# kubeai-project/kubeai

Measured on AMD Instinct MI355X. Metric: output_tokens_per_s (k6 multi-turn chat), higher is better.
Workload: dtype fp8; 1 GPU; model=llama-3-8b, global_batch=40, seq_len=8192, parallelism=dp1, prefix_cache=True

## Files before the change

### kubeai_amd/csrc/attention_decode.hip

```cpp
#include <torch/extension.h>

#include <type_traits>

#include "attention_checks.h"
#include "attention_plan.h"
#include "common.h"
#include "dispatch.h"

namespace {

constexpr int kWaves = 2;
constexpr int kBlockThreads = kWaves * WAVE_SIZE;
constexpr int kBS = 16;
typedef __attribute__((ext_vector_type(2))) __bf16 bf16x2v;
constexpr int kPad = 8;

template <int G, typename CT = ushort, int HD = 128, bool CAP = false,
          bool RAW = false>
__launch_bounds__(kBlockThreads) __global__ void paged_decode_kernel(
    ushort* __restrict__ out,
    const ushort* __restrict__ q,
    std::conditional_t<RAW, CT*, const CT*> __restrict__ k_cache,
    std::conditional_t<RAW, CT*, const CT*> __restrict__ v_cache,
    const int32_t* __restrict__ block_tables,
    const int32_t* __restrict__ seq_lens,
    const float scale, const float softcap, const int window,
    const int n_kv, const int max_blocks,
    const int64_t q_stride, const int n_splits,
    float* __restrict__ part_o,
    float* __restrict__ part_ml,
    const ushort* __restrict__ k_new,
    const ushort* __restrict__ v_new,
    const int32_t* __restrict__ positions,
    const float* __restrict__ cos_sin,
    const int64_t* __restrict__ slot_mapping,
    const int64_t k_stride, const int64_t v_stride) {
  const int b = blockIdx.x / (n_kv * n_splits);
  const int rem = blockIdx.x % (n_kv * n_splits);
  const int kh = rem / n_splits;
  const int split = rem % n_splits;
  const int n_q = n_kv * G;
  const int wave = threadIdx.x / WAVE_SIZE;
  const int lane = threadIdx.x % WAVE_SIZE;
  const int L = seq_lens[b];
  int pos = 0;
  int64_t slot = -1;
  if constexpr (RAW) {
    pos = positions[b];
    slot = slot_mapping[b];
  }
  const int n_blocks = (L + kBS - 1) / kBS;
  const int w0 = (window > 0) ? max(0, L - window) : 0;
  const int blk_base = w0 / kBS;
  const int n_eff = n_blocks - blk_base;
  const int chunk = (n_eff + n_splits - 1) / n_splits;
  const int blk_lo = blk_base + split * chunk;
  const int blk_hi = min(n_blocks, blk_lo + chunk);

  constexpr int PARTS = HD / 32;
  constexpr int TOKP = 64 / PARTS;
  constexpr int EPL = HD / 64;
  __shared__ CT k_lds[kWaves][kBS][HD + kPad];
  __shared__ CT v_lds[kWaves][kBS][HD + kPad];
  __shared__ float merge_o[kWaves][G][HD];
  __shared__ float merge_ml[kWaves][G][2];

  const int tok_of = lane / PARTS;
  const int part = lane % PARTS;

  uint32_t q_pack[G][16];
  if constexpr (!RAW) {
#pragma unroll
    for (int g = 0; g < G; ++g) {
      const uint32_t* qp = reinterpret_cast<const uint32_t*>(
          q + (int64_t)b * q_stride + (int64_t)(kh * G + g) * HD + part * 32);
#pragma unroll
      for (int i = 0; i < 16; ++i) q_pack[g][i] = qp[i];
    }
  }

  const int32_t* bt = block_tables + (int64_t)b * max_blocks;
  const int first = blk_lo + wave;
  int64_t blk_first = 0;
  if constexpr (RAW) blk_first = bt[first < blk_hi ? first : 0];

  constexpr int HALF = HD / 2;
  constexpr int QV = G * HALF / 4;
  constexpr int QIT = (QV + WAVE_SIZE - 1) / WAVE_SIZE;
  ushort4_t q_lo[RAW ? QIT : 1], q_hi[RAW ? QIT : 1];
  float4_t q_c[RAW ? QIT : 1], q_s[RAW ? QIT : 1];
  constexpr int RV = HD / 8;
  ushort8 row_own, row_par;
  float4_t row_c[2], row_s[2];
  const bool row_hi = (lane % RV) >= RV / 2;
  if constexpr (RAW) {
    const float* cs = cos_sin + (int64_t)pos * HD;
#pragma unroll
    for (int it = 0; it < QIT; ++it) {
      const int idx = lane + it * WAVE_SIZE;
      if (QV % WAVE_SIZE == 0 || idx < QV) {
        const int g = idx / (HALF / 4);
        const int i = (idx % (HALF / 4)) * 4;
        const ushort* qh =
            q + (int64_t)b * q_stride + (int64_t)(kh * G + g) * HD + i;
        q_lo[it] = *reinterpret_cast<const ushort4_t*>(qh);
        q_hi[it] = *reinterpret_cast<const ushort4_t*>(qh + HALF);
        q_c[it] = *reinterpret_cast<const float4_t*>(cs + i);
        q_s[it] = *reinterpret_cast<const float4_t*>(cs + HALF + i);
      }
    }
    {
      const int e0 = (lane % RV) * 8;
      const ushort* row = ((lane / RV) % 2 == 0
                               ? k_new + (int64_t)b * k_stride
                               : v_new + (int64_t)b * v_stride) +
                          (int64_t)kh * HD;
      row_own = *reinterpret_cast<const ushort8*>(row + e0);
      row_par = *reinterpret_cast<const ushort8*>(
          row + (row_hi ? e0 - HALF : e0 + HALF));
      const int i = row_hi ? e0 - HALF : e0;
#pragma unroll
      for (int h = 0; h < 2; ++h) {
        row_c[h] = *reinterpret_cast<const float4_t*>(cs + i + 4 * h);
        row_s[h] = *reinterpret_cast<const float4_t*>(cs + HALF + i + 4 * h);
      }
    }
  }

  float m[G], l[G], o[G][EPL];
#pragma unroll
  for (int g = 0; g < G; ++g) {
    m[g] = -INFINITY;
    l[g] = 0.f;
#pragma unroll
    for (int e = 0; e < EPL; ++e) o[g][e] = 0.f;
  }

  using StageVec = std::conditional_t<sizeof(CT) == 2, ushort8, uint64_t>;
  constexpr int NS = (kBS * HD / 8) / WAVE_SIZE;
  StageVec stage_k[NS], stage_v[NS];
  typedef StageVec __attribute__((may_alias)) LdsVec;

  auto issue_tile = [&](const int64_t blk) {
    const CT* base_k = k_cache + ((blk * n_kv + kh) * kBS) * HD;
    const CT* base_v = v_cache + ((blk * n_kv + kh) * kBS) * HD;
    const StageVec* src_k = reinterpret_cast<const StageVec*>(base_k);
    const StageVec* src_v = reinterpret_cast<const StageVec*>(base_v);
#pragma unroll
    for (int i = 0; i < NS; ++i) {
      stage_k[i] = src_k[lane + i * WAVE_SIZE];
      stage_v[i] = src_v[lane + i * WAVE_SIZE];
    }
  };
  auto issue_loads = [&](int blk_i) { issue_tile(bt[blk_i]); };
  auto write_tile = [&]() {
#pragma unroll
    for (int i = 0; i < NS; ++i) {
      const int vec = lane + i * WAVE_SIZE;
      const int row = vec / (HD / 8);
      const int col = vec % (HD / 8);
      *reinterpret_cast<LdsVec*>(&k_lds[wave][row][col * 8]) = stage_k[i];
      *reinterpret_cast<LdsVec*>(&v_lds[wave][row][col * 8]) = stage_v[i];
    }
  };

  if (first < blk_hi) {
    if constexpr (RAW)
      issue_tile(blk_first);
    else
      issue_loads(first);
  }

  int row_blk = -1;
  StageVec row_vec{};
  if constexpr (RAW) {
    ushort* q_rot = reinterpret_cast<ushort*>(&merge_o[wave][0][0]);
#pragma unroll
    for (int it = 0; it < QIT; ++it) {
      const int idx = lane + it * WAVE_SIZE;
      if (QV % WAVE_SIZE == 0 || idx < QV) {
        const int g = idx / (HALF / 4);
        const int i = (idx % (HALF / 4)) * 4;
        ushort4_t r_lo, r_hi;
#pragma unroll
        for (int e = 0; e < 4; ++e) {
          ushort o1, o2;
          rope_rotate_pair(bf16_to_f32(q_lo[it][e]), bf16_to_f32(q_hi[it][e]),
                           q_c[it][e], q_s[it][e], o1, o2);
          r_lo[e] = o1;
          r_hi[e] = o2;
        }
        *reinterpret_cast<ushort4_t*>(q_rot + g * HD + i) = r_lo;
        *reinterpret_cast<ushort4_t*>(q_rot + g * HD + HALF + i) = r_hi;
      }
    }
#pragma unroll
    for (int g = 0; g < G; ++g) {
      const uint4* qp =
          reinterpret_cast<const uint4*>(q_rot + g * HD + part * 32);
#pragma unroll
      for (int i = 0; i < 4; ++i) {
        const uint4 t = qp[i];
        q_pack[g][4 * i] = t.x;
        q_pack[g][4 * i + 1] = t.y;
        q_pack[g][4 * i + 2] = t.z;
        q_pack[g][4 * i + 3] = t.w;
      }
    }

    const int new_blk = (L - 1) / kBS;
    const bool owner = slot >= 0 && L > 0 && new_blk >= blk_lo &&
                       new_blk < blk_hi && (new_blk - blk_lo) % kWaves == wave;
    if (owner) {
      row_blk = new_blk;
      if (lane < 2 * RV) {
        ushort8 row = row_own;
        if (lane < RV) {
#pragma unroll
          for (int e = 0; e < 8; ++e) {
            const float x_own = bf16_to_f32(row_own[e]);
            const float x_par = bf16_to_f32(row_par[e]);
            ushort o1, o2;
            rope_rotate_pair(row_hi ? x_par : x_own, row_hi ? x_own : x_par,
                             row_c[e / 4][e % 4], row_s[e / 4][e % 4], o1, o2);
            row[e] = row_hi ? o2 : o1;
          }
        }
        if constexpr (sizeof(CT) == 2) {
          row_vec = row;
        } else {
          row_vec = 0;
#pragma unroll
          for (int e = 0; e < 8; ++e)
            row_vec |= (uint64_t)f32_to_e5m2(bf16_to_f32((ushort)row[e]))
                       << (8 * e);
        }
        CT* dst = (lane < RV ? k_cache : v_cache) +
                  cache_row_offset(slot, kBS, n_kv, kh, HD) + (lane % RV) * 8;
        *reinterpret_cast<StageVec*>(dst) = row_vec;
      }
    }
  }
  if (first < blk_hi) write_tile();

  for (int blk_i = first; blk_i < blk_hi; blk_i += kWaves) {
    const int tile_start = blk_i * kBS;
    const int tile_len = min(kBS, L - tile_start);
    if (blk_i + kWaves < blk_hi) issue_loads(blk_i + kWaves);

    if constexpr (RAW) {
      if (blk_i == row_blk && lane < 2 * RV) {
        CT* dst = lane < RV ? &k_lds[wave][(L - 1) % kBS][lane * 8]
                            : &v_lds[wave][(L - 1) % kBS][(lane - RV) * 8];
        *reinterpret_cast<LdsVec*>(dst) = row_vec;
      }
    }

#pragma unroll
    for (int tp = 0; tp < kBS; tp += TOKP) {
      const int tok = tp + tok_of;
      float s[G];
#pragma unroll
      for (int g = 0; g < G; ++g) s[g] = 0.f;
      if constexpr (sizeof(CT) == 2) {
        const uint32_t* krow = reinterpret_cast<const uint32_t*>(
            &k_lds[wave][tok][part * 32]);
#pragma unroll
        for (int j = 0; j < 16; ++j) {
          const bf16x2v kk = __builtin_bit_cast(bf16x2v, krow[j]);
#pragma unroll
          for (int g = 0; g < G; ++g)
            s[g] = __builtin_amdgcn_fdot2_f32_bf16(
                kk, __builtin_bit_cast(bf16x2v, q_pack[g][j]), s[g], false);
        }
      } else {
        const uint32_t* krow = reinterpret_cast<const uint32_t*>(
            &k_lds[wave][tok][part * 32]);
#pragma unroll
        for (int j = 0; j < 8; ++j) {
          const uint32_t kk = krow[j];
          const floatx2 k01 = __builtin_amdgcn_cvt_pk_f32_bf8(kk, false);
          const floatx2 k23 = __builtin_amdgcn_cvt_pk_f32_bf8(kk, true);
#pragma unroll
          for (int g = 0; g < G; ++g) {
            const uint32_t qa = q_pack[g][2 * j];
            const uint32_t qb = q_pack[g][2 * j + 1];
            s[g] = fmaf(k01.x, bf16_to_f32((ushort)(qa & 0xffff)), s[g]);
            s[g] = fmaf(k01.y, bf16_to_f32((ushort)(qa >> 16)), s[g]);
            s[g] = fmaf(k23.x, bf16_to_f32((ushort)(qb & 0xffff)), s[g]);
            s[g] = fmaf(k23.y, bf16_to_f32((ushort)(qb >> 16)), s[g]);
          }
        }
      }
      float p[G];
      float rsum[G];
#pragma unroll
      for (int g = 0; g < G; ++g) {
#pragma unroll
        for (int off = 1; off < PARTS; off <<= 1)
          s[g] += __shfl_xor(s[g], off, 64);
        s[g] = (tok < tile_len && tile_start + tok >= w0) ? s[g] * scale
                                                          : -INFINITY;
        if constexpr (CAP) {
          if (s[g] != -INFINITY) s[g] = softcap * tanhf(s[g] / softcap);
        }
        float tmax = s[g];
#pragma unroll
        for (int off = PARTS; off < 64; off <<= 1)
          tmax = fmaxf(tmax, __shfl_xor(tmax, off, 64));
        const float m_new = fmaxf(m[g], tmax);
        if (m_new != m[g]) {
          const float corr = __expf(m[g] - m_new);
          l[g] *= corr;
#pragma unroll
          for (int e = 0; e < EPL; ++e) o[g][e] *= corr;
          m[g] = m_new;
        }
        p[g] = (s[g] == -INFINITY) ? 0.f : __expf(s[g] - m_new);
        rsum[g] = p[g];
#pragma unroll
        for (int off = 1; off < 64; off <<= 1)
          rsum[g] += __shfl_xor(rsum[g], off, 64);
        l[g] += rsum[g] * (1.0f / PARTS);
      }

#pragma unroll
      for (int t = tp; t < tp + TOKP; ++t) {
        if (t >= tile_len) break;
        float vv[EPL];
        if constexpr (sizeof(CT) == 2) {
#pragma unroll
          for (int e = 0; e < EPL; e += 2) {
            const uint32_t vr = *reinterpret_cast<const uint32_t*>(
                &v_lds[wave][t][EPL * lane + e]);
            vv[e] = bf16_to_f32((ushort)(vr & 0xffff));
            vv[e + 1] = bf16_to_f32((ushort)(vr >> 16));
          }
        } else {
#pragma unroll
          for (int e = 0; e < EPL; e += 2) {
            const uint32_t vr = *reinterpret_cast<const ushort*>(
                &v_lds[wave][t][EPL * lane + e]);
            const floatx2 vf = __builtin_amdgcn_cvt_pk_f32_bf8(vr, false);
            vv[e] = vf.x;
            vv[e + 1] = vf.y;
          }
        }
#pragma unroll
        for (int g = 0; g < G; ++g) {
          const float pt = __shfl(p[g], (t - tp) * PARTS, 64);
#pragma unroll
          for (int e = 0; e < EPL; ++e)
            o[g][e] = fmaf(pt, vv[e], o[g][e]);
        }
      }
    }

    if (blk_i + kWaves < blk_hi) write_tile();
  }

#pragma unroll
  for (int g = 0; g < G; ++g) {
#pragma unroll
    for (int e = 0; e < EPL; ++e) merge_o[wave][g][EPL * lane + e] = o[g][e];
    if (lane == 0) {
      merge_ml[wave][g][0] = m[g];
      merge_ml[wave][g][1] = l[g];
    }
  }
  __syncthreads();

  for (int g = wave; g < G; g += kWaves) {
    float m_star = -INFINITY;
#pragma unroll
    for (int w = 0; w < kWaves; ++w) m_star = fmaxf(m_star, merge_ml[w][g][0]);
    float l_star = 0.f, oo[EPL];
#pragma unroll
    for (int e = 0; e < EPL; ++e) oo[e] = 0.f;
    if (m_star != -INFINITY) {
#pragma unroll
      for (int w = 0; w < kWaves; ++w) {
        const float c = __expf(merge_ml[w][g][0] - m_star);
        l_star += merge_ml[w][g][1] * c;
#pragma unroll
        for (int e = 0; e < EPL; ++e)
          oo[e] += merge_o[w][g][EPL * lane + e] * c;
      }
    }
    const int head = kh * G + g;
    if (n_splits == 1) {
      const float inv_l = 1.0f / l_star;
      ushort* oh = out + ((int64_t)b * n_q + head) * HD;
#pragma unroll
      for (int e = 0; e < EPL; e += 2) {
        uint32_t packed =
            ((uint32_t)f32_to_bf16(oo[e + 1] * inv_l) << 16) |
            f32_to_bf16(oo[e] * inv_l);
        *reinterpret_cast<uint32_t*>(&oh[EPL * lane + e]) = packed;
      }
    } else {
      float* po = part_o + (((int64_t)b * n_q + head) * n_splits + split) * HD;
#pragma unroll
      for (int e = 0; e < EPL; ++e) po[EPL * lane + e] = oo[e];
      if (lane == 0) {
        float* pm = part_ml + (((int64_t)b * n_q + head) * n_splits + split) * 2;
        pm[0] = m_star;
        pm[1] = l_star;
      }
    }
  }
}

constexpr int kMergeSplitCapLo = 8;
constexpr int kMergeSplitCapHi = 16;

template <int N, int HD, int SCAP>
DEV_INLINE void merge_partials(const float* __restrict__ po,
                               const float* __restrict__ pml,
                               const int n_splits, uint32_t (&packed)[N / 2]) {
  typedef float __attribute__((ext_vector_type(N))) vecN;
  floatx2 ml[SCAP];
  vecN pv[SCAP];
#pragma unroll
  for (int s = 0; s < SCAP; ++s) {
    const int sc = min(s, n_splits - 1);
    ml[s] = *reinterpret_cast<const floatx2*>(pml + 2 * sc);
    pv[s] = *reinterpret_cast<const vecN*>(po + sc * HD);
  }
  __builtin_amdgcn_sched_barrier(0);
  float m_star = -INFINITY;
#pragma unroll
  for (int s = 0; s < SCAP; ++s)
    if (s < n_splits) m_star = fmaxf(m_star, ml[s].x);
  float l_star = 0.f, oo[N];
#pragma unroll
  for (int e = 0; e < N; ++e) oo[e] = 0.f;
#pragma unroll
  for (int s = 0; s < SCAP; ++s) {
    const bool use = s < n_splits && ml[s].x != -INFINITY;
    const float c = __expf(ml[s].x - m_star);
    l_star = use ? l_star + ml[s].y * c : l_star;
#pragma unroll
    for (int e = 0; e < N; ++e) oo[e] = use ? oo[e] + pv[s][e] * c : oo[e];
  }
  const float inv_l = 1.0f / l_star;
#pragma unroll
  for (int e = 0; e < N; e += 2)
    packed[e / 2] = ((uint32_t)f32_to_bf16(oo[e + 1] * inv_l) << 16) |
                    f32_to_bf16(oo[e] * inv_l);
}

template <int HD, int SCAP>
__global__ void decode_merge_kernel(
    ushort* __restrict__ out,
    const float* __restrict__ part_o,
    const float* __restrict__ part_ml,
    const int n_q, const int n_splits, const int64_t n_bh) {
  constexpr int EPL = HD / 64;
  const int64_t bh = (int64_t)blockIdx.x * (blockDim.x / WAVE_SIZE) +
                     threadIdx.x / WAVE_SIZE;
  if (bh >= n_bh) return;
  const int lane = threadIdx.x % WAVE_SIZE;
  uint32_t packed[EPL / 2];
  merge_partials<EPL, HD, SCAP>(part_o + bh * n_splits * HD + EPL * lane,
                                part_ml + bh * n_splits * 2, n_splits, packed);
  ushort* oh = out + bh * HD;
#pragma unroll
  for (int e = 0; e < EPL; e += 2)
    *reinterpret_cast<uint32_t*>(&oh[EPL * lane + e]) = packed[e / 2];
}

constexpr int kMergeVec = 4;
constexpr int kMergeMaxThreads = 1024;
constexpr int kMergeMaxPasses = 2;
constexpr int kMergeRowMax = kMergeMaxThreads * kMergeVec * kMergeMaxPasses;

template <int HD, int kPasses, int SCAP>
__launch_bounds__(kMergeMaxThreads) __global__ void decode_merge_fp8_kernel(
    ushort* __restrict__ out,
    unsigned char* __restrict__ out_fp8,
    float* __restrict__ out_scale,
    const float* __restrict__ part_o,
    const float* __restrict__ part_ml,
    const int n_q, const int n_splits) {
  __shared__ float red[16];
  const int b = blockIdx.x;
  const int row_len = n_q * HD;
  const int nvec = row_len / kMergeVec;
  ushort* orow = out + (int64_t)b * row_len;

  uint32_t packed[kPasses][kMergeVec / 2];
  float amax = 0.f;
#pragma unroll
  for (int it = 0; it < kPasses; ++it) {
    const int i = threadIdx.x + it * blockDim.x;
    if (i < nvec) {
      const int h = (i * kMergeVec) / HD;
      const int col = (i * kMergeVec) % HD;
      const int64_t bh = (int64_t)b * n_q + h;
      merge_partials<kMergeVec, HD, SCAP>(part_o + bh * n_splits * HD + col,
                                          part_ml + bh * n_splits * 2,
                                          n_splits, packed[it]);
      *reinterpret_cast<uint2*>(orow + i * kMergeVec) =
          make_uint2(packed[it][0], packed[it][1]);
#pragma unroll
      for (int e = 0; e < kMergeVec / 2; ++e) {
        const uint32_t pk = packed[it][e];
        amax = fmaxf(amax, fabsf(bf16_to_f32((ushort)(pk & 0xffff))));
        amax = fmaxf(amax, fabsf(bf16_to_f32((ushort)(pk >> 16))));
      }
    }
  }
  const float inv_scale = row_scale_fp8(amax, red, out_scale + b);
  unsigned char* frow = out_fp8 + (int64_t)b * row_len;
#pragma unroll
  for (int it = 0; it < kPasses; ++it) {
    const int i = threadIdx.x + it * blockDim.x;
    if (i < nvec) {
      uchar4 q4;
      const uint32_t p0 = packed[it][0], p1 = packed[it][1];
      q4.x = f32_to_fp8(bf16_to_f32((ushort)(p0 & 0xffff)) * inv_scale);
      q4.y = f32_to_fp8(bf16_to_f32((ushort)(p0 >> 16)) * inv_scale);
      q4.z = f32_to_fp8(bf16_to_f32((ushort)(p1 & 0xffff)) * inv_scale);
      q4.w = f32_to_fp8(bf16_to_f32((ushort)(p1 >> 16)) * inv_scale);
      *reinterpret_cast<uchar4*>(frow + i * kMergeVec) = q4;
    }
  }
}

}

void quant_fp8(torch::Tensor out, torch::Tensor out_scale, torch::Tensor x);

namespace {

struct RawQKV {
  torch::Tensor k, v, positions, cos_sin, slot_mapping;
};

void decode_impl(torch::Tensor out, const c10::optional<torch::Tensor>& out_fp8,
                 const c10::optional<torch::Tensor>& out_scale, torch::Tensor q,
                 torch::Tensor k_cache, torch::Tensor v_cache,
                 torch::Tensor block_tables, torch::Tensor seq_lens,
                 double scale, int64_t window, double softcap,
                 const RawQKV* raw = nullptr) {
  const AttnShape s =
      check_paged_attention(out, q, k_cache, v_cache, block_tables, seq_lens);
  const int B = q.size(0), n_q = s.n_q, n_kv = s.n_kv, hd = s.hd;
  const int max_blocks = s.max_blocks;
  TORCH_CHECK(seq_lens.numel() >= B && block_tables.size(0) >= B);
  const bool want_fp8 = out_fp8.has_value();
  if (want_fp8) {
    TORCH_CHECK(out_scale.has_value());
    check_fp8_out(out, *out_fp8, *out_scale);
  }
  const ushort *k_new = nullptr, *v_new = nullptr;
  const int32_t* positions = nullptr;
  const float* cos_sin = nullptr;
  const int64_t* slot_mapping = nullptr;
  int64_t k_stride = 0, v_stride = 0;
  if (raw != nullptr) {
    const torch::Tensor &k = raw->k, &v = raw->v;
    TORCH_CHECK(k.dim() == 3 && v.dim() == 3);
    TORCH_CHECK(k.scalar_type() == torch::kBFloat16 &&
                v.scalar_type() == torch::kBFloat16);
    TORCH_CHECK(k.size(0) == B && k.size(1) == n_kv && k.size(2) == hd);
    TORCH_CHECK(v.size(0) == B && v.size(1) == n_kv && v.size(2) == hd);
    TORCH_CHECK(k.stride(2) == 1 && k.stride(1) == hd);
    TORCH_CHECK(v.stride(2) == 1 && v.stride(1) == hd);
    TORCH_CHECK(v_cache.sizes() == k_cache.sizes() &&
                v_cache.scalar_type() == k_cache.scalar_type());
    TORCH_CHECK(k_cache.size(3) == hd);
    TORCH_CHECK(raw->positions.scalar_type() == torch::kInt32 &&
                raw->positions.is_contiguous() && raw->positions.numel() >= B);
    TORCH_CHECK(raw->slot_mapping.scalar_type() == torch::kInt64 &&
                raw->slot_mapping.is_contiguous() &&
                raw->slot_mapping.numel() >= B);
    TORCH_CHECK(raw->cos_sin.scalar_type() == torch::kFloat32 &&
                raw->cos_sin.dim() == 2 && raw->cos_sin.size(1) == hd &&
                raw->cos_sin.is_contiguous());
    auto aligned = [](const torch::Tensor& t, int64_t bytes) {
      return reinterpret_cast<uintptr_t>(t.data_ptr()) % bytes == 0 &&
             (t.dim() < 3 || t.stride(0) * t.element_size() % bytes == 0);
    };
    TORCH_CHECK(aligned(q, 8) && aligned(k, 16) && aligned(v, 16) &&
                    aligned(raw->cos_sin, 16) && aligned(k_cache, 16) &&
                    aligned(v_cache, 16),
                "rope_cache_attention_decode: misaligned q/k/v/cos_sin/cache");
    k_new = (const ushort*)k.data_ptr();
    v_new = (const ushort*)v.data_ptr();
    positions = raw->positions.data_ptr<int32_t>();
    cos_sin = raw->cos_sin.data_ptr<float>();
    slot_mapping = raw->slot_mapping.data_ptr<int64_t>();
    k_stride = k.stride(0);
    v_stride = v.stride(0);
  }
  if (B == 0) return;
  const int n_splits = attn_plan::decode_n_splits(B, n_kv, max_blocks);
  torch::Tensor part_o, part_ml;
  float *part_o_ptr = nullptr, *part_ml_ptr = nullptr;
  if (n_splits > 1) {
    auto opts =
        torch::TensorOptions().device(q.device()).dtype(torch::kFloat32);
    part_o = torch::empty({B, n_q, n_splits, (int64_t)hd}, opts);
    part_ml = torch::empty({B, n_q, n_splits, 2}, opts);
    part_o_ptr = part_o.data_ptr<float>();
    part_ml_ptr = part_ml.data_ptr<float>();
  }
  dim3 grid(B * n_kv * n_splits), block(kBlockThreads);
  auto stream = c10::hip::getCurrentHIPStream().stream();
  dispatch_int<1, 2, 4, 5, 6, 8>(s.G, "GQA group size", [&](auto g) {
    dispatch_int<128, 256>(hd, "head dim", [&](auto hdv) {
      dispatch_bool(s.fp8_cache, [&](auto fp8) {
        dispatch_bool(softcap > 0.0, [&](auto cap) {
          dispatch_bool(raw != nullptr, [&](auto rawv) {
            using CT = std::conditional_t<decltype(fp8)::value, unsigned char,
                                          ushort>;
            hipLaunchKernelGGL(
                (paged_decode_kernel<decltype(g)::value, CT,
                                     decltype(hdv)::value, decltype(cap)::value,
                                     decltype(rawv)::value>),
                grid, block, 0, stream, (ushort*)out.data_ptr(),
                (const ushort*)q.data_ptr(), (CT*)k_cache.data_ptr(),
                (CT*)v_cache.data_ptr(), block_tables.data_ptr<int32_t>(),
                seq_lens.data_ptr<int32_t>(), (float)scale, (float)softcap,
                (int)window, n_kv, max_blocks, q.stride(0), n_splits,
                part_o_ptr, part_ml_ptr, k_new, v_new, positions, cos_sin,
                slot_mapping, k_stride, v_stride);
          });
        });
      });
    });
  });
  HIP_CHECK_KERNEL();
  if (n_splits == 1) {
    if (want_fp8) quant_fp8(*out_fp8, *out_scale, out.view({B, -1}));
    return;
  }
  static_assert(kMergeSplitCapHi == 16, "decode_n_splits caps splits at 16");
  TORCH_CHECK(n_splits <= kMergeSplitCapHi);
  const bool fuse_fp8 = want_fp8 && (int64_t)n_q * hd <= kMergeRowMax;
  dispatch_int<128, 256>(hd, "head dim", [&](auto hdv) {
    dispatch_bool(n_splits <= kMergeSplitCapLo, [&](auto lo) {
      constexpr int HD = decltype(hdv)::value;
      constexpr int SCAP =
          decltype(lo)::value ? kMergeSplitCapLo : kMergeSplitCapHi;
      if (fuse_fp8) {
        const int nvec = n_q * hd / kMergeVec;
        const int threads = std::min(
            kMergeMaxThreads, (nvec + WAVE_SIZE - 1) / WAVE_SIZE * WAVE_SIZE);
        dispatch_int<1, 2>(
            (nvec + threads - 1) / threads, "merge pass count", [&](auto p) {
              hipLaunchKernelGGL(
                  (decode_merge_fp8_kernel<HD, decltype(p)::value, SCAP>),
                  dim3(B), dim3(threads), 0, stream, (ushort*)out.data_ptr(),
                  (unsigned char*)out_fp8->data_ptr(),
                  out_scale->data_ptr<float>(), part_o_ptr, part_ml_ptr, n_q,
                  n_splits);
            });
      } else {
        const int64_t n_bh = (int64_t)B * n_q;
        const int wpb = 4;
        hipLaunchKernelGGL((decode_merge_kernel<HD, SCAP>),
                           dim3((uint32_t)((n_bh + wpb - 1) / wpb)),
                           dim3(wpb * WAVE_SIZE), 0, stream,
                           (ushort*)out.data_ptr(), part_o_ptr, part_ml_ptr,
                           n_q, n_splits, n_bh);
      }
    });
  });
  HIP_CHECK_KERNEL();
  if (want_fp8 && !fuse_fp8) quant_fp8(*out_fp8, *out_scale, out.view({B, -1}));
}

}

void paged_attention_decode(torch::Tensor out, torch::Tensor q,
                            torch::Tensor k_cache, torch::Tensor v_cache,
                            torch::Tensor block_tables, torch::Tensor seq_lens,
                            double scale, int64_t window, double softcap) {
  decode_impl(out, c10::nullopt, c10::nullopt, q, k_cache, v_cache,
              block_tables, seq_lens, scale, window, softcap);
}

void paged_attention_decode_fp8(torch::Tensor out, torch::Tensor out_fp8,
                                torch::Tensor out_scale, torch::Tensor q,
                                torch::Tensor k_cache, torch::Tensor v_cache,
                                torch::Tensor block_tables,
                                torch::Tensor seq_lens, double scale,
                                int64_t window, double softcap) {
  decode_impl(out, out_fp8, out_scale, q, k_cache, v_cache, block_tables,
              seq_lens, scale, window, softcap);
}

void rope_cache_attention_decode(
    torch::Tensor out, c10::optional<torch::Tensor> out_fp8,
    c10::optional<torch::Tensor> out_scale, torch::Tensor q, torch::Tensor k,
    torch::Tensor v, torch::Tensor positions, torch::Tensor cos_sin,
    torch::Tensor k_cache, torch::Tensor v_cache, torch::Tensor slot_mapping,
    torch::Tensor block_tables, torch::Tensor seq_lens, double scale,
    int64_t window, double softcap) {
  const RawQKV raw{k, v, positions, cos_sin, slot_mapping};
  decode_impl(out, out_fp8, out_scale, q, k_cache, v_cache, block_tables,
              seq_lens, scale, window, softcap, &raw);
}
```

### kubeai_amd/csrc/bindings.cpp

```cpp
#include <torch/extension.h>

#include <tuple>
#include <utility>

#include "attention_plan.h"

void rmsnorm(torch::Tensor out, torch::Tensor x, torch::Tensor weight,
             double eps);
void fused_add_rmsnorm(torch::Tensor x, torch::Tensor residual,
                       torch::Tensor weight, double eps);
void rope(torch::Tensor q, torch::Tensor k, torch::Tensor positions,
          torch::Tensor cos_sin);
void rope_and_cache(torch::Tensor q, torch::Tensor k, torch::Tensor v,
                    torch::Tensor positions, torch::Tensor cos_sin,
                    torch::Tensor k_cache, torch::Tensor v_cache,
                    torch::Tensor slot_mapping);
void reshape_and_cache(torch::Tensor k, torch::Tensor v, torch::Tensor k_cache,
                       torch::Tensor v_cache, torch::Tensor slot_mapping);
void paged_attention_decode(torch::Tensor out, torch::Tensor q,
                            torch::Tensor k_cache, torch::Tensor v_cache,
                            torch::Tensor block_tables, torch::Tensor seq_lens,
                            double scale, int64_t window, double softcap);
void paged_attention_decode_fp8(torch::Tensor out, torch::Tensor out_fp8,
                                torch::Tensor out_scale, torch::Tensor q,
                                torch::Tensor k_cache, torch::Tensor v_cache,
                                torch::Tensor block_tables,
                                torch::Tensor seq_lens, double scale,
                                int64_t window, double softcap);
void rope_cache_attention_decode(
    torch::Tensor out, c10::optional<torch::Tensor> out_fp8,
    c10::optional<torch::Tensor> out_scale, torch::Tensor q, torch::Tensor k,
    torch::Tensor v, torch::Tensor positions, torch::Tensor cos_sin,
    torch::Tensor k_cache, torch::Tensor v_cache, torch::Tensor slot_mapping,
    torch::Tensor block_tables, torch::Tensor seq_lens, double scale,
    int64_t window, double softcap);
void paged_attention_prefill(torch::Tensor out, torch::Tensor q,
                             torch::Tensor k_cache, torch::Tensor v_cache,
                             torch::Tensor block_tables,
                             torch::Tensor query_start_loc,
                             torch::Tensor seq_lens, double scale,
                             int64_t window, double softcap);
void silu_and_mul(torch::Tensor out, torch::Tensor x);
void gelu_and_mul(torch::Tensor out, torch::Tensor x);
void skinny_gemm(torch::Tensor y, torch::Tensor x, torch::Tensor w);
void int4_dequant(torch::Tensor out, torch::Tensor qp, torch::Tensor sp,
                  torch::Tensor zp, int64_t N, int64_t K, int64_t group);
void int4_gemm(torch::Tensor y, torch::Tensor x, torch::Tensor qp,
               torch::Tensor sp, torch::Tensor zp, int64_t N, int64_t K,
               int64_t group);
int64_t int4_gemm_tiles(int64_t N, int64_t M);
void int4_moe_gemm(torch::Tensor y, torch::Tensor x, torch::Tensor selected,
                   torch::Tensor table, int64_t row_div, int64_t E, int64_t N,
                   int64_t K, int64_t group, int64_t n_tiles);
void moe_combine(torch::Tensor out, torch::Tensor y, torch::Tensor selected,
                 torch::Tensor weights, int64_t E);
std::tuple<int64_t, int64_t> int4_moe_plan(int64_t N, int64_t T, int64_t E,
                                           int64_t k);
void greedy_sample(torch::Tensor out, torch::Tensor logits);
void gumbel_sample(torch::Tensor out, torch::Tensor logits,
                   torch::Tensor temperature, torch::Tensor seeds,
                   int64_t step);
void greedy_sample_logprob(torch::Tensor out, torch::Tensor out_logprob,
                           torch::Tensor out_lse, torch::Tensor logits);
void gumbel_sample_logprob(torch::Tensor out, torch::Tensor out_logprob,
                           torch::Tensor out_lse, torch::Tensor logits,
                           torch::Tensor temperature, torch::Tensor seeds,
                           int64_t step);
void token_logprobs(torch::Tensor out_logprob, torch::Tensor out_lse,
                    torch::Tensor logits, torch::Tensor tokens);
void sgmv(torch::Tensor y, torch::Tensor x, torch::Tensor A, torch::Tensor B,
          torch::Tensor idx, double scale);
void register_chwbl(pybind11::module_& m);
pybind11::bytes xgmi_alloc();
void xgmi_connect(int64_t rank, int64_t world,
                  const std::vector<pybind11::bytes>& handles);
void xgmi_fused_allreduce_add_rmsnorm(torch::Tensor x, torch::Tensor residual,
                                      torch::Tensor weight, double eps);
int64_t xgmi_error_count();
int64_t xgmi_max_elems();
void xgmi_shutdown();
void rmsnorm_fp8(torch::Tensor out, torch::Tensor out_scale, torch::Tensor x,
                 torch::Tensor weight, double eps);
void fused_add_rmsnorm_fp8(torch::Tensor out, torch::Tensor out_scale,
                           torch::Tensor x, torch::Tensor residual,
                           torch::Tensor weight, double eps);
void fused_add_rmsnorm_fp8_div(torch::Tensor out, torch::Tensor out_scale,
                               torch::Tensor x, torch::Tensor residual,
                               torch::Tensor weight, double eps,
                               bool write_rows);
void embed_rmsnorm_fp8(torch::Tensor out, torch::Tensor out_scale,
                       torch::Tensor x_out, torch::Tensor ids,
                       torch::Tensor table, torch::Tensor weight, double eps);
void silu_and_mul_fp8(torch::Tensor out, torch::Tensor out_scale,
                      torch::Tensor x);
void quant_fp8(torch::Tensor out, torch::Tensor out_scale, torch::Tensor x);
void quant_fp8_div(torch::Tensor out, torch::Tensor out_scale,
                   torch::Tensor x);
void nucleus_stats(torch::Tensor m, torch::Tensor z, torch::Tensor logits,
                   torch::Tensor temps);
void nucleus_accept(torch::Tensor ok, torch::Tensor logits,
                    torch::Tensor cand, torch::Tensor m, torch::Tensor z,
                    torch::Tensor temps, torch::Tensor top_ps,
                    torch::Tensor top_ks);

static std::pair<int64_t, int64_t> prefill_plan(int64_t Tq, int64_t B,
                                                int64_t n_q, int64_t n_kv,
                                                int64_t hd, int64_t max_blocks,
                                                int64_t window,
                                                double softcap) {
  TORCH_CHECK(n_kv > 0 && n_q % n_kv == 0);
  const attn_plan::PrefillPlan p = attn_plan::prefill_plan(
      Tq, (int)B, (int)n_q, (int)n_kv, (int)hd, (int)max_blocks, window,
      softcap);
  return {p.version, p.waves};
}
static int64_t decode_plan(int64_t B, int64_t n_kv, int64_t max_blocks) {
  return attn_plan::decode_n_splits((int)B, (int)n_kv, (int)max_blocks);
}

PYBIND11_MODULE(TORCH_EXTENSION_NAME, m) {
  m.def("prefill_plan", &prefill_plan,
        "(version, waves per workgroup) paged_attention_prefill launches",
        pybind11::arg("Tq"), pybind11::arg("B"), pybind11::arg("n_q"),
        pybind11::arg("n_kv"), pybind11::arg("hd"),
        pybind11::arg("max_blocks"), pybind11::arg("window") = 0,
        pybind11::arg("softcap") = 0.0);
  m.def("decode_plan", &decode_plan,
        "flash-decoding splits paged_attention_decode launches",
        pybind11::arg("B"), pybind11::arg("n_kv"),
        pybind11::arg("max_blocks"));
  m.def("rmsnorm", &rmsnorm, "RMSNorm (bf16, fp32 accum)");
  m.def("fused_add_rmsnorm", &fused_add_rmsnorm,
        "in-place residual add + RMSNorm");
  m.def("rope", &rope, "NeoX rotary embedding, in-place q/k");
  m.def("rope_and_cache", &rope_and_cache,
        "rotary embedding (in-place q/k) fused with the paged KV cache write");
  m.def("reshape_and_cache", &reshape_and_cache,
        "paged KV cache write (bf16 or fp8 e5m2 cache)");
  m.def("paged_attention_decode", &paged_attention_decode,
        "paged attention, one query token per seq");
  m.def("paged_attention_decode_fp8", &paged_attention_decode_fp8,
        "paged decode attention that also emits the e4m3 row quant of out");
  m.def("rope_cache_attention_decode", &rope_cache_attention_decode,
        "pure-decode step: rotary embedding and KV cache write inside the "
        "decode attention kernel (q, k, v are only read)");
  m.def("paged_attention_prefill", &paged_attention_prefill,
        "paged causal flash attention over cached KV");
  m.def("gelu_and_mul", &gelu_and_mul, "GeGLU tanh-gelu(gate)*up");
  m.def("silu_and_mul", &silu_and_mul, "SwiGLU activation");
  m.def("skinny_gemm", &skinny_gemm, "weight-streaming GEMM for M<=64");
  m.def("int4_dequant", &int4_dequant,
        "packed int4 weight -> bf16 [N, K], bit-equal to Int4Weight.dequant()");
  m.def("int4_gemm", &int4_gemm,
        "fused dequant + GEMM over a packed int4 weight, M <= 64");
  m.def("int4_gemm_tiles", &int4_gemm_tiles,
        "16-column tiles per workgroup int4_gemm launches with",
        pybind11::arg("N"), pybind11::arg("M"));
  m.def("int4_moe_gemm", &int4_moe_gemm,
        "y[t*k+j] = x[(t*k+j) / row_div] @ W[selected[t,j]]^T over packed int4 "
        "experts, T <= 64; n_tiles = 0 takes int4_moe_plan's",
        pybind11::arg("y"), pybind11::arg("x"), pybind11::arg("selected"),
        pybind11::arg("table"), pybind11::arg("row_div"), pybind11::arg("E"),
        pybind11::arg("N"), pybind11::arg("K"), pybind11::arg("group"),
        pybind11::arg("n_tiles") = 0);
  m.def("moe_combine", &moe_combine,
        "out[t] = sum_j weights[t,j] * y[t*k+j] in ascending expert id, bf16 "
        "steps; ids outside [0, E) are skipped (E = 0: no upper limit)",
        pybind11::arg("out"), pybind11::arg("y"), pybind11::arg("selected"),
        pybind11::arg("weights"), pybind11::arg("E") = 0);
  m.def("int4_moe_plan", &int4_moe_plan,
        "(16-row tiles, 16-column tiles per workgroup) int4_moe_gemm launches "
        "with", pybind11::arg("N"), pybind11::arg("T"), pybind11::arg("E"),
        pybind11::arg("k"));
  m.def("greedy_sample", &greedy_sample, "argmax sampling");
  m.def("gumbel_sample", &gumbel_sample, "temperature sampling (hash RNG)");
  m.def("greedy_sample_logprob", &greedy_sample_logprob,
        "argmax sampling + the token's logprob and the row logsumexp");
  m.def("gumbel_sample_logprob", &gumbel_sample_logprob,
        "temperature sampling + the token's logprob and the row logsumexp");
  m.def("token_logprobs", &token_logprobs,
        "logprob of given tokens and the row logsumexp, one launch");
  m.def("rmsnorm_fp8", &rmsnorm_fp8, "rmsnorm with fused fp8 row quant");
  m.def("fused_add_rmsnorm_fp8", &fused_add_rmsnorm_fp8,
        "residual add + rmsnorm with fused fp8 row quant");
  m.def("fused_add_rmsnorm_fp8_div", &fused_add_rmsnorm_fp8_div,
        "residual add + rmsnorm, then the division-form fp8 row quant of its "
        "bf16 row (lm_head's input)");
  m.def("embed_rmsnorm_fp8", &embed_rmsnorm_fp8,
        "embedding gather + rmsnorm with fused fp8 row quant (layer 0)");
  m.def("silu_and_mul_fp8", &silu_and_mul_fp8, "SwiGLU with fused fp8 quant");
  m.def("quant_fp8", &quant_fp8, "bf16 -> fp8 row quant");
  m.def("quant_fp8_div", &quant_fp8_div,
        "bf16 -> fp8 row quant, division form (Fp8Linear.forward)");
  m.def("nucleus_stats", &nucleus_stats, "per-row softmax max + Z");
  m.def("nucleus_accept", &nucleus_accept,
        "nucleus membership of sampled tokens (mass above < p, rank < k)");
  m.def("xgmi_alloc", &xgmi_alloc, "allocate + export the IPC comm buffer");
  m.def("xgmi_connect", &xgmi_connect, "open peer IPC buffers");
  m.def("xgmi_fused_allreduce_add_rmsnorm", &xgmi_fused_allreduce_add_rmsnorm,
        "one-shot xGMI all-reduce fused with residual add + RMSNorm");
  m.def("xgmi_error_count", &xgmi_error_count, "spin-wait timeout count");
  m.def("xgmi_max_elems", &xgmi_max_elems, "one-shot capacity (bf16 elems)");
  m.def("xgmi_shutdown", &xgmi_shutdown, "free/close comm buffers");
  m.def("sgmv", &sgmv, "segmented gather LoRA apply (one adapter segment)");
  register_chwbl(m);
}
```

### kubeai_amd/csrc/common.h

```cpp
#pragma once

#include <hip/hip_runtime.h>
#include <hip/hip_bf16.h>
#include <hip/hip_fp16.h>
#include <hip/hip_fp8.h>
#include <stdint.h>
#include <c10/hip/HIPStream.h>

#define WAVE_SIZE 64
#define DEV_INLINE __device__ __forceinline__

typedef __hip_bfloat16 bf16_t;

typedef ushort __attribute__((ext_vector_type(8))) ushort8;
typedef ushort __attribute__((ext_vector_type(4))) ushort4_t;
typedef float __attribute__((ext_vector_type(4))) float4_t;

DEV_INLINE float bf16_to_f32(ushort u) {
  union {
    uint32_t i;
    float f;
  } c;
  c.i = ((uint32_t)u) << 16;
  return c.f;
}

DEV_INLINE ushort f32_to_bf16(float f) {
  union {
    float f;
    uint32_t i;
  } c;
  c.f = f;
  uint32_t x = c.i;
  uint32_t rb = ((x >> 16) & 1u) + 0x7fffu;
  x += rb;
  return (ushort)(x >> 16);
}


DEV_INLINE float e5m2_to_f32(unsigned char b) {
  const uint32_t s = ((uint32_t)b & 0x80u) << 24;
  uint32_t e = (b >> 2) & 0x1fu;
  uint32_t m = b & 0x3u;
  uint32_t out;
  if (e == 0) {
    if (m == 0) {
      out = s;
    } else {
      int shift = (m & 2u) ? 0 : 1;
      e = 127 - 15 + 1 - 1 - shift;
      m = (m << (shift + 1)) & 0x3u;
      out = s | (e << 23) | (m << 21);
    }
  } else if (e == 0x1fu) {
    out = s | 0x7f800000u | (m << 21);
  } else {
    out = s | ((e - 15u + 127u) << 23) | (m << 21);
  }
  union { uint32_t i; float f; } c;
  c.i = out;
  return c.f;
}

typedef float floatx2 __attribute__((ext_vector_type(2)));

DEV_INLINE ushort8 e5m2x8_to_bf16x8(uint64_t raw) {
  ushort8 out;
#pragma unroll
  for (int j = 0; j < 8; ++j) {
    const ushort h = (ushort)((raw >> (8 * j)) << 8);
    const float f = __half2float(__builtin_bit_cast(__half, h));
    out[j] = (ushort)(__builtin_bit_cast(uint32_t, f) >> 16);
  }
  return out;
}

DEV_INLINE unsigned char f32_to_e5m2(float x) {
  return (unsigned char)__hip_cvt_float_to_fp8(x, __HIP_SATFINITE, __HIP_E5M2);
}

DEV_INLINE uint64_t bf16x8_to_e5m2x8(const ushort8 v) {
  uint64_t out = 0;
#pragma unroll
  for (int j = 0; j < 8; ++j)
    out |= (uint64_t)f32_to_e5m2(bf16_to_f32((ushort)v[j])) << (8 * j);
  return out;
}

DEV_INLINE int64_t cache_row_offset(const int64_t slot, const int bs,
                                    const int n_kv, const int head,
                                    const int hd) {
  return (((slot / bs) * n_kv + head) * bs + slot % bs) * hd;
}

DEV_INLINE void rope_rotate_pair(const float x1, const float x2, const float c,
                                 const float s, ushort& o1, ushort& o2) {
#pragma clang fp contract(off)
  const float x2s = x2 * s;
  const float x2c = x2 * c;
  o1 = f32_to_bf16(__builtin_fmaf(x1, c, -x2s));
  o2 = f32_to_bf16(__builtin_fmaf(x1, s, x2c));
}


DEV_INLINE float wave_reduce_sum(float v) {
#pragma unroll
  for (int off = 32; off > 0; off >>= 1) v += __shfl_xor(v, off, 64);
  return v;
}

DEV_INLINE float wave_reduce_max(float v) {
#pragma unroll
  for (int off = 32; off > 0; off >>= 1) v = fmaxf(v, __shfl_xor(v, off, 64));
  return v;
}

DEV_INLINE float block_reduce_sum(float v, float* smem) {
  const int wave = threadIdx.x / WAVE_SIZE;
  const int lane = threadIdx.x % WAVE_SIZE;
  const int n_waves = (blockDim.x + WAVE_SIZE - 1) / WAVE_SIZE;
  v = wave_reduce_sum(v);
  if (lane == 0) smem[wave] = v;
  __syncthreads();
  float total = 0.f;
#pragma unroll
  for (int w = 0; w < 16; ++w)
    if (w < n_waves) total += smem[w];
  return total;
}

DEV_INLINE float block_amax(float v, float* smem) {
  const int wave = threadIdx.x / WAVE_SIZE;
  const int lane = threadIdx.x % WAVE_SIZE;
  const int n_waves = (blockDim.x + WAVE_SIZE - 1) / WAVE_SIZE;
  v = wave_reduce_max(v);
  if (lane == 0) smem[wave] = v;
  __syncthreads();
  float m = 0.f;
#pragma unroll
  for (int w = 0; w < 16; ++w)
    if (w < n_waves) m = fmaxf(m, smem[w]);
  return m;
}

DEV_INLINE unsigned char f32_to_fp8(float x) {
  return (unsigned char)__hip_cvt_float_to_fp8(x, __HIP_SATFINITE, __HIP_E4M3);
}

DEV_INLINE uint2 quant8_fp8(const float (&f)[8], const float inv_scale) {
  uchar2 packed[4];
#pragma unroll
  for (int j = 0; j < 4; ++j) {
    packed[j].x = f32_to_fp8(f[2 * j] * inv_scale);
    packed[j].y = f32_to_fp8(f[2 * j + 1] * inv_scale);
  }
  return *reinterpret_cast<uint2*>(packed);
}

DEV_INLINE float row_scale_fp8(const float amax, float* smem,
                               float* __restrict__ scale_out) {
  const float gmax = fmaxf(block_amax(amax, smem), 1e-6f);
  if (threadIdx.x == 0) *scale_out = gmax / 448.0f;
  return 448.0f / gmax;
}

DEV_INLINE float row_scale_fp8_div(const float amax, float* smem,
                                   float* __restrict__ scale_out) {
  const float gmax = fmaxf(block_amax(amax, smem), 1e-6f);
  const float scale = gmax * (float)(1.0 / 448.0);
  if (threadIdx.x == 0) *scale_out = scale;
  return scale;
}

DEV_INLINE uint2 quant8_fp8_div(const float (&f)[8], const float scale) {
  uchar2 packed[4];
#pragma unroll
  for (int j = 0; j < 4; ++j) {
    packed[j].x =
        f32_to_fp8(fminf(fmaxf(f[2 * j] / scale, -448.0f), 448.0f));
    packed[j].y =
        f32_to_fp8(fminf(fmaxf(f[2 * j + 1] / scale, -448.0f), 448.0f));
  }
  return *reinterpret_cast<uint2*>(packed);
}

DEV_INLINE float silu(const float x) { return x / (1.0f + __expf(-x)); }

DEV_INLINE uint64_t splitmix64(uint64_t z) {
  z += 0x9e3779b97f4a7c15ull;
  z = (z ^ (z >> 30)) * 0xbf58476d1ce4e5b9ull;
  z = (z ^ (z >> 27)) * 0x94d049bb133111ebull;
  return z ^ (z >> 31);
}

DEV_INLINE float hash_uniform(uint64_t key, uint64_t idx) {
  uint64_t h = splitmix64(key ^ (idx * 0xd1342543de82ef95ull));
  uint32_t m = (uint32_t)(h >> 40);
  return ((float)m + 1.0f) * (1.0f / 16777216.0f);
}

#define HIP_CHECK_KERNEL()                                    \
  do {                                                        \
    hipError_t e = hipGetLastError();                         \
    if (e != hipSuccess) {                                    \
      TORCH_CHECK(false, "HIP kernel launch failed: ",        \
                  hipGetErrorString(e));                      \
    }                                                         \
  } while (0)
```

### kubeai_amd/csrc/row_kernels.hip

```cpp
#include <torch/extension.h>

#include <type_traits>

#include "common.h"
#include "dispatch.h"

namespace {

constexpr int kBlock = 256;
constexpr int kBlockWide = 512;
constexpr int kMaxIters = 8;
constexpr int kMaxH = kBlockWide * 8 * kMaxIters;

template <int kThreads, int kIters, bool kDiv = false>
DEV_INLINE void store_row_fp8(unsigned char* __restrict__ orow,
                              const float (&vals)[kIters][8],
                              const float factor, const int nvec) {
#pragma unroll
  for (int it = 0; it < kIters; ++it) {
    const int i = threadIdx.x + it * kThreads;
    if (i < nvec)
      *reinterpret_cast<uint2*>(orow + i * 8) =
          kDiv ? quant8_fp8_div(vals[it], factor) : quant8_fp8(vals[it], factor);
  }
}

template <bool kFused, bool kFp8Out, int kThreads, int kIters,
          bool kDiv = false, bool kEmbed = false>
__launch_bounds__(kThreads) __global__ void rmsnorm_kernel(
    std::conditional_t<kFp8Out, unsigned char, ushort>* __restrict__ out,
    float* __restrict__ out_scale,
    ushort* __restrict__ x,
    ushort* __restrict__ residual,
    const ushort* __restrict__ w,
    const float eps, const int H,
    const int32_t* __restrict__ ids = nullptr,
    const int V = 0,
    const bool write_rows = true) {
  static_assert(!kEmbed || (kFp8Out && !kFused && !kDiv));
  static_assert(!kDiv || (kFp8Out && kFused));
  const int row = blockIdx.x;
  int64_t src = row;
  if constexpr (kEmbed) src = min(max(ids[row], 0), V - 1);
  ushort8* xrow = reinterpret_cast<ushort8*>(x + src * H);
  ushort8* rrow = (kFused || kEmbed)
                      ? reinterpret_cast<ushort8*>(residual + (int64_t)row * H)
                      : nullptr;
  const ushort8* wv = reinterpret_cast<const ushort8*>(w);
  const int nvec = H / 8;

  float vals[kIters][8];
  float ssum = 0.f;
#pragma unroll
  for (int it = 0; it < kIters; ++it) {
    const int i = threadIdx.x + it * kThreads;
    if (i < nvec) {
      ushort8 xv = xrow[i];
      ushort8 rin;
      if constexpr (kFused) rin = rrow[i];
#pragma unroll
      for (int j = 0; j < 8; ++j) {
        float f = bf16_to_f32(xv[j]);
        if constexpr (kFused) f += bf16_to_f32(rin[j]);
        vals[it][j] = f;
        ssum += f * f;
      }
      if constexpr (kFused) {
        if (!kDiv || write_rows) {
          ushort8 rv;
#pragma unroll
          for (int j = 0; j < 8; ++j) rv[j] = f32_to_bf16(vals[it][j]);
          rrow[i] = rv;
        }
      }
      if constexpr (kEmbed) rrow[i] = xv;
    }
  }
  ushort8 wreg[kIters];
#pragma unroll
  for (int it = 0; it < kIters; ++it) {
    const int i = threadIdx.x + it * kThreads;
    if (i < nvec) wreg[it] = wv[i];
  }

  __shared__ float red[16];
  const float total = block_reduce_sum(ssum, red);
  const float inv_rms = rsqrtf(total / (float)H + eps);

  if constexpr (kDiv) {
    float amax = 0.f;
#pragma unroll
    for (int it = 0; it < kIters; ++it) {
      const int i = threadIdx.x + it * kThreads;
      if (i < nvec) {
        ushort8 ov;
#pragma unroll
        for (int j = 0; j < 8; ++j) {
          ov[j] = f32_to_bf16(vals[it][j] * inv_rms * bf16_to_f32(wreg[it][j]));
          vals[it][j] = bf16_to_f32(ov[j]);
          amax = fmaxf(amax, fabsf(vals[it][j]));
        }
        if (write_rows) xrow[i] = ov;
      }
    }
    __syncthreads();
    const float scale = row_scale_fp8_div(amax, red, out_scale + row);
    store_row_fp8<kThreads, kIters, true>(out + (int64_t)row * H, vals, scale,
                                          nvec);
  } else if constexpr (kFp8Out) {
    float amax = 0.f;
#pragma unroll
    for (int it = 0; it < kIters; ++it) {
      const int i = threadIdx.x + it * kThreads;
      if (i < nvec) {
#pragma unroll
        for (int j = 0; j < 8; ++j) {
          vals[it][j] *= inv_rms * bf16_to_f32(wreg[it][j]);
          amax = fmaxf(amax, fabsf(vals[it][j]));
        }
      }
    }
    __syncthreads();
    const float inv_scale = row_scale_fp8(amax, red, out_scale + row);
    store_row_fp8<kThreads, kIters>(out + (int64_t)row * H, vals, inv_scale,
                                    nvec);
  } else {
    ushort8* orow = reinterpret_cast<ushort8*>(out + (int64_t)row * H);
#pragma unroll
    for (int it = 0; it < kIters; ++it) {
      const int i = threadIdx.x + it * kThreads;
      if (i < nvec) {
        ushort8 ov;
#pragma unroll
        for (int j = 0; j < 8; ++j)
          ov[j] = f32_to_bf16(vals[it][j] * inv_rms * bf16_to_f32(wreg[it][j]));
        orow[i] = ov;
      }
    }
  }
}

struct LoadBf16 {
  static constexpr int kInWidth = 1;
  DEV_INLINE static void load(const ushort* __restrict__ in, const int W,
                              const int i, float (&v)[8]) {
    const ushort8 xv = reinterpret_cast<const ushort8*>(in)[i];
#pragma unroll
    for (int j = 0; j < 8; ++j) v[j] = bf16_to_f32(xv[j]);
  }
};

struct LoadSwiglu {
  static constexpr int kInWidth = 2;
  DEV_INLINE static void load(const ushort* __restrict__ in, const int W,
                              const int i, float (&v)[8]) {
    const ushort8 g = reinterpret_cast<const ushort8*>(in)[i];
    const ushort8 u = reinterpret_cast<const ushort8*>(in + W)[i];
#pragma unroll
    for (int j = 0; j < 8; ++j) v[j] = silu(bf16_to_f32(g[j])) * bf16_to_f32(u[j]);
  }
};

template <typename Producer, bool kDiv, int kThreads, int kIters>
__launch_bounds__(kThreads) __global__ void row_fp8_kernel(
    unsigned char* __restrict__ out,
    float* __restrict__ out_scale,
    const ushort* __restrict__ xin,
    const int W) {
  const int row = blockIdx.x;
  const ushort* in = xin + (int64_t)row * Producer::kInWidth * W;
  const int nvec = W / 8;

  float vals[kIters][8];
  float amax = 0.f;
#pragma unroll
  for (int it = 0; it < kIters; ++it) {
    const int i = threadIdx.x + it * kThreads;
    if (i < nvec) {
      Producer::load(in, W, i, vals[it]);
#pragma unroll
      for (int j = 0; j < 8; ++j) amax = fmaxf(amax, fabsf(vals[it][j]));
    }
  }
  __shared__ float red[16];
  const float factor = kDiv ? row_scale_fp8_div(amax, red, out_scale + row)
                            : row_scale_fp8(amax, red, out_scale + row);
  store_row_fp8<kThreads, kIters, kDiv>(out + (int64_t)row * W, vals, factor,
                                        nvec);
}

enum class RowPolicy { kNorm, kMax };

template <RowPolicy kPolicy, typename Launch>
void dispatch_row(const int nvec, Launch&& launch) {
  if (nvec <= kBlock) {
    launch(Int<kBlock>{}, Int<1>{});
  } else if (nvec <= kBlock * 2) {
    launch(Int<kBlock>{}, Int<2>{});
  } else if (nvec <= kBlock * 4) {
    launch(Int<kBlock>{}, Int<4>{});
  } else if constexpr (kPolicy == RowPolicy::kNorm) {
    if (nvec <= kBlock * kMaxIters) launch(Int<kBlock>{}, Int<kMaxIters>{});
    else launch(Int<kBlockWide>{}, Int<kMaxIters>{});
  } else {
    if (nvec <= kBlockWide * 4) launch(Int<kBlockWide>{}, Int<4>{});
    else launch(Int<kBlockWide>{}, Int<kMaxIters>{});
  }
}

void check_row_op(const torch::Tensor& x, const int64_t W) {
  TORCH_CHECK(x.is_contiguous());
  TORCH_CHECK(x.scalar_type() == torch::kBFloat16);
  TORCH_CHECK(W % 8 == 0 && W <= kMaxH);
}

template <bool kFused, bool kFp8Out, bool kDiv = false, bool kEmbed = false>
void launch_rmsnorm(void* out, float* out_scale, const torch::Tensor& x,
                    void* residual, const torch::Tensor& weight, double eps,
                    const torch::Tensor* ids = nullptr,
                    const bool write_rows = true) {
  const int H = x.size(-1);
  check_row_op(x, H);
  const int T = kEmbed ? ids->numel() : x.numel() / H;
  if constexpr (kDiv || kEmbed) {
    TORCH_CHECK(weight.is_contiguous() && weight.numel() == H &&
                weight.scalar_type() == torch::kBFloat16);
    if (T == 0) return;
  }
  using out_t = std::conditional_t<kFp8Out, unsigned char, ushort>;
  dispatch_row<RowPolicy::kNorm>(H / 8, [&](auto threads, auto iters) {
    constexpr int kThreads = decltype(threads)::value;
    constexpr int kIters = decltype(iters)::value;
    hipLaunchKernelGGL(
        (rmsnorm_kernel<kFused, kFp8Out, kThreads, kIters, kDiv, kEmbed>),
        dim3(T), dim3(kThreads), 0, c10::hip::getCurrentHIPStream().stream(),
        (out_t*)out, out_scale, (ushort*)x.data_ptr(), (ushort*)residual,
        (const ushort*)weight.data_ptr(), (float)eps, H,
        kEmbed ? ids->data_ptr<int32_t>() : nullptr,
        kEmbed ? (int)x.size(0) : 0, write_rows);
  });
  HIP_CHECK_KERNEL();
}

template <typename Producer, bool kDiv = false>
void launch_row_fp8(torch::Tensor& out, torch::Tensor& out_scale,
                    const torch::Tensor& x) {
  const int W = x.size(-1) / Producer::kInWidth;
  check_row_op(x, W);
  TORCH_CHECK(x.size(-1) == (int64_t)W * Producer::kInWidth);
  const int T = x.numel() / x.size(-1);
  if (T == 0) return;
  dispatch_row<RowPolicy::kMax>(W / 8, [&](auto threads, auto iters) {
    constexpr int kThreads = decltype(threads)::value;
    constexpr int kIters = decltype(iters)::value;
    hipLaunchKernelGGL((row_fp8_kernel<Producer, kDiv, kThreads, kIters>), dim3(T),
                       dim3(kThreads), 0,
                       c10::hip::getCurrentHIPStream().stream(),
                       (unsigned char*)out.data_ptr(),
                       out_scale.data_ptr<float>(),
                       (const ushort*)x.data_ptr(), W);
  });
  HIP_CHECK_KERNEL();
}

}

void rmsnorm(torch::Tensor out, torch::Tensor x, torch::Tensor weight,
             double eps) {
  TORCH_CHECK(out.is_contiguous());
  launch_rmsnorm<false, false>(out.data_ptr(), nullptr, x, nullptr, weight, eps);
}

void fused_add_rmsnorm(torch::Tensor x, torch::Tensor residual,
                       torch::Tensor weight, double eps) {
  TORCH_CHECK(residual.is_contiguous());
  launch_rmsnorm<true, false>(x.data_ptr(), nullptr, x, residual.data_ptr(),
                              weight, eps);
}

void rmsnorm_fp8(torch::Tensor out, torch::Tensor out_scale, torch::Tensor x,
                 torch::Tensor weight, double eps) {
  launch_rmsnorm<false, true>(out.data_ptr(), out_scale.data_ptr<float>(), x,
                              nullptr, weight, eps);
}

void fused_add_rmsnorm_fp8(torch::Tensor out, torch::Tensor out_scale,
                           torch::Tensor x, torch::Tensor residual,
                           torch::Tensor weight, double eps) {
  TORCH_CHECK(residual.is_contiguous());
  launch_rmsnorm<true, true>(out.data_ptr(), out_scale.data_ptr<float>(), x,
                             residual.data_ptr(), weight, eps);
}

void fused_add_rmsnorm_fp8_div(torch::Tensor out, torch::Tensor out_scale,
                               torch::Tensor x, torch::Tensor residual,
                               torch::Tensor weight, double eps,
                               bool write_rows) {
  TORCH_CHECK(residual.is_contiguous() && residual.sizes() == x.sizes() &&
              residual.scalar_type() == torch::kBFloat16);
  TORCH_CHECK(out.is_contiguous() && out.numel() == x.numel() &&
              out.element_size() == 1);
  TORCH_CHECK(out_scale.is_contiguous() &&
              out_scale.scalar_type() == torch::kFloat32 &&
              out_scale.numel() * x.size(-1) == x.numel());
  launch_rmsnorm<true, true, true>(out.data_ptr(), out_scale.data_ptr<float>(),
                                   x, residual.data_ptr(), weight, eps, nullptr,
                                   write_rows);
}

void embed_rmsnorm_fp8(torch::Tensor out, torch::Tensor out_scale,
                       torch::Tensor x_out, torch::Tensor ids,
                       torch::Tensor table, torch::Tensor weight, double eps) {
  TORCH_CHECK(table.dim() == 2 && table.size(0) >= 1);
  TORCH_CHECK(ids.dim() == 1 && ids.is_contiguous() &&
              ids.scalar_type() == torch::kInt32);
  const int64_t T = ids.numel(), H = table.size(1);
  TORCH_CHECK(x_out.is_contiguous() && x_out.dim() == 2 && x_out.size(0) == T &&
              x_out.size(1) == H && x_out.scalar_type() == torch::kBFloat16);
  TORCH_CHECK(out.is_contiguous() && out.numel() == T * H &&
              out.element_size() == 1);
  TORCH_CHECK(out_scale.is_contiguous() &&
              out_scale.scalar_type() == torch::kFloat32 &&
              out_scale.numel() == T);
  launch_rmsnorm<false, true, false, true>(
      out.data_ptr(), out_scale.data_ptr<float>(), table, x_out.data_ptr(),
      weight, eps, &ids);
}

void silu_and_mul_fp8(torch::Tensor out, torch::Tensor out_scale,
                      torch::Tensor x) {
  launch_row_fp8<LoadSwiglu>(out, out_scale, x);
}

void quant_fp8(torch::Tensor out, torch::Tensor out_scale, torch::Tensor x) {
  launch_row_fp8<LoadBf16>(out, out_scale, x);
}

void quant_fp8_div(torch::Tensor out, torch::Tensor out_scale,
                   torch::Tensor x) {
  launch_row_fp8<LoadBf16, true>(out, out_scale, x);
}
```

### kubeai_amd/models/llama.py

```python
from __future__ import annotations

import math

import torch
import torch.nn as nn
import torch.nn.functional as F

from kubeai_amd import ops
from kubeai_amd.engine.batch import ForwardBatch
from .config import ModelArchConfig


class EngineLinear(nn.Linear):

    def forward(self, x: torch.Tensor) -> torch.Tensor:
        y = ops.linear(x, self.weight)
        if self.bias is not None:
            y = y + self.bias
        return y


def _rms_head(x: torch.Tensor, w: torch.Tensor, eps: float) -> torch.Tensor:
    if x.is_cuda and x.dtype == torch.bfloat16:
        flat = x.contiguous().view(-1, x.shape[-1])
        return ops.rmsnorm(flat, w, eps).view(x.shape)
    xf = x.float()
    xf = xf * torch.rsqrt(xf.pow(2).mean(-1, keepdim=True) + eps)
    return (xf * w.float()).to(x.dtype)


def paged_attention_step(
    q: torch.Tensor,
    k: torch.Tensor,
    v: torch.Tensor,
    fb: ForwardBatch,
    kv_cache: tuple[torch.Tensor, torch.Tensor],
    cos_sin: torch.Tensor,
    *,
    scale: float,
    window: int,
    softcap: float,
    fp8_out: bool,
):
    k_cache, v_cache = kv_cache
    T = q.shape[0]
    out = torch.empty(q.shape, dtype=q.dtype, device=q.device)
    nd = fb.n_decode
    if fb.n_prefill == 0 and nd == T and nd > 0 and q.is_cuda:
        res = ops.rope_cache_attention_decode(
            q,
            k,
            v,
            fb.positions,
            cos_sin,
            k_cache,
            v_cache,
            fb.slot_mapping,
            fb.decode_block_tables,
            fb.decode_seq_lens,
            scale,
            out=out,
            window=window,
            softcap=softcap,
            fp8_out=fp8_out,
        )
        return res[1:] if fp8_out else out.view(T, -1)
    q, k = ops.rope_and_cache(
        q, k, v, fb.positions, cos_sin, k_cache, v_cache, fb.slot_mapping
    )
    if nd > 0:
        ops.paged_attention_decode(
            q[:nd],
            k_cache,
            v_cache,
            fb.decode_block_tables,
            fb.decode_seq_lens,
            scale,
            out=out[:nd],
            window=window,
            softcap=softcap,
        )
    if fb.n_prefill > 0:
        ops.paged_attention_prefill(
            q[nd:],
            k_cache,
            v_cache,
            fb.prefill_block_tables,
            fb.prefill_query_start_loc,
            fb.prefill_seq_lens,
            scale,
            out=out[nd:],
            window=window,
            softcap=softcap,
        )
    attn_flat = out.view(T, -1)
    return ops.quant_fp8(attn_flat) if fp8_out else attn_flat


class Attention(nn.Module):
    def __init__(self, cfg: ModelArchConfig, layer_idx: int):
        super().__init__()
        self.layer_idx = layer_idx
        self.n_q = cfg.num_attention_heads
        self.n_kv = cfg.num_key_value_heads
        self.hd = cfg.head_dim
        if cfg.global_layer_interval > 0:
            self.is_global = (layer_idx + 1) % cfg.global_layer_interval == 0
            use_win = not self.is_global
        else:
            self.is_global = True
            use_win = (
                cfg.sliding_window_pattern != "even" or layer_idx % 2 == 0
            )
        self.window = (cfg.sliding_window or 0) if use_win else 0
        self.qk_norm = cfg.qk_norm
        if cfg.qk_norm:
            self.q_norm = nn.Parameter(torch.ones(cfg.head_dim))
            self.k_norm = nn.Parameter(torch.ones(cfg.head_dim))
        self.norm_eps = cfg.rms_norm_eps
        self.softcap = cfg.attn_logit_softcap or 0.0
        self.scale = (
            cfg.attention_multiplier
            or 1.0 / math.sqrt(cfg.query_pre_attn_scalar or self.hd)
        )
        q_size = self.n_q * self.hd
        kv_size = self.n_kv * self.hd
        self.qkv_proj = EngineLinear(
            cfg.hidden_size, q_size + 2 * kv_size, bias=cfg.attention_bias
        )
        self.o_proj = EngineLinear(q_size, cfg.hidden_size, bias=False)

    def forward(
        self,
        x: torch.Tensor,
        fb: ForwardBatch,
        kv_cache: tuple[torch.Tensor, torch.Tensor],
        cos_sin: torch.Tensor,
    ) -> torch.Tensor:
        fp8_in = isinstance(x, tuple)
        if fp8_in:
            xq, xs = x
            qkv = self.qkv_proj.forward_quantized(xq, xs)
            lm = None
        else:
            qkv = self.qkv_proj(x)
            lm = getattr(self, "_lora_manager", None)
            if lm is not None and lm.active and fb.lora_ids is not None:
                lm.apply(self.layer_idx, "qkv", x, qkv, fb.lora_ids)
        q, k, v = qkv.split(
            [self.n_q * self.hd, self.n_kv * self.hd, self.n_kv * self.hd], dim=-1
        )
        q = q.unflatten(-1, (self.n_q, self.hd))
        k = k.unflatten(-1, (self.n_kv, self.hd))
        v = v.unflatten(-1, (self.n_kv, self.hd))
        if self.qk_norm:
            q = _rms_head(q, self.q_norm, self.norm_eps)
            k = _rms_head(k, self.k_norm, self.norm_eps)
        if isinstance(cos_sin, tuple):
            cos_sin = cos_sin[0] if self.is_global else cos_sin[1]
        attn = paged_attention_step(
            q, k, v, fb, kv_cache, cos_sin, scale=self.scale,
            window=self.window, softcap=self.softcap, fp8_out=fp8_in,
        )
        if fp8_in:
            return self.o_proj.forward_quantized(*attn)
        return self._o_proj_bf16(attn, fb, lm)

    def _o_proj_bf16(self, attn_flat, fb: ForwardBatch, lm) -> torch.Tensor:
        result = self.o_proj(attn_flat)
        if lm is not None and lm.active and fb.lora_ids is not None:
            lm.apply(self.layer_idx, "o", attn_flat, result, fb.lora_ids)
        return result


class MLP(nn.Module):
    def __init__(self, cfg: ModelArchConfig, layer_idx: int | None = None):
        super().__init__()
        self.layer_idx = layer_idx
        self.gate_up_proj = EngineLinear(
            cfg.hidden_size, 2 * cfg.intermediate_size, bias=False
        )
        self.down_proj = EngineLinear(cfg.intermediate_size, cfg.hidden_size, bias=False)
        self.gelu = cfg.hidden_act == "gelu_pytorch_tanh"

    def forward(self, x, fb: ForwardBatch | None = None) -> torch.Tensor:
        if isinstance(x, tuple):
            h = self.gate_up_proj.forward_quantized(*x)
            a8, ascale = ops.silu_and_mul_fp8(h)
            return self.down_proj.forward_quantized(a8, ascale)
        h = self.gate_up_proj(x)
        lm = getattr(self, "_lora_manager", None)
        lora_live = (
            lm is not None and lm.active and fb is not None
            and fb.lora_ids is not None and self.layer_idx is not None
        )
        if lora_live:
            lm.apply(self.layer_idx, "gate_up", x, h, fb.lora_ids)
        a = ops.gelu_and_mul(h) if self.gelu else ops.silu_and_mul(h)
        y = self.down_proj(a)
        if lora_live:
            lm.apply(self.layer_idx, "down", a, y, fb.lora_ids)
        return y


class MoEMLP(nn.Module):

    def __init__(self, cfg: ModelArchConfig):
        super().__init__()
        self.n_experts = cfg.num_local_experts
        self.top_k = cfg.num_experts_per_tok
        self.gate = nn.Linear(cfg.hidden_size, self.n_experts, bias=False)
        self.experts = nn.ModuleList([MLP(cfg) for _ in range(self.n_experts)])
        self._int4_groups = None

    def _apply(self, fn, *args, **kwargs):
        super()._apply(fn, *args, **kwargs)
        self.refresh_int4_groups()
        return self

    def refresh_int4_groups(self):
        self._int4_groups = None
        if not any(ex.gelu for ex in self.experts):
            from kubeai_amd.engine.quant_int4 import expert_groups

            self._int4_groups = expert_groups(self.experts)
        return self._int4_groups

    def int4_groups(self):
        groups = self._int4_groups
        if groups is not None and not (
            groups[0].holds([ex.gate_up_proj for ex in self.experts])
            and groups[1].holds([ex.down_proj for ex in self.experts])
        ):
            groups = self.refresh_int4_groups()
        return groups

    def forward(self, x: torch.Tensor, fb: ForwardBatch | None = None) -> torch.Tensor:
        T, H = x.shape
        router = F.linear(x.float(), self.gate.weight.float())
        weights, selected = torch.topk(router, self.top_k, dim=-1)
        weights = torch.softmax(weights, dim=-1).to(x.dtype)
        if x.is_cuda and 1 <= T <= min(ops.INT4_MOE_T, 64):
            groups = self.int4_groups()
            if groups is not None:
                return ops.int4_moe_mlp(x, selected, weights, *groups)
        if T <= 256:
            wfull = torch.zeros(T, self.n_experts, dtype=x.dtype,
                                device=x.device)
            wfull.scatter_(1, selected, weights)
            fp8 = hasattr(self.experts[0].gate_up_proj, "forward_quantized")
            if fp8:
                xq, xs = ops.quant_fp8(x)
            out = None
            for e in range(self.n_experts):
                contrib = (
                    self.experts[e]((xq, xs)) if fp8 else self.experts[e](x)
                )
                contrib = contrib * wfull[:, e : e + 1]
                out = contrib if out is None else out + contrib
            return out
        fp8 = hasattr(self.experts[0].gate_up_proj, "forward_quantized")
        if fp8:
            xq, xs = ops.quant_fp8(x)
            xq_bytes = xq.view(torch.uint8)
        out = torch.zeros_like(x)
        for e in range(self.n_experts):
            mask = selected == e
            tok_idx, k_idx = mask.nonzero(as_tuple=True)
            if tok_idx.numel() == 0:
                continue
            if fp8:
                sub = (xq_bytes[tok_idx].view(xq.dtype), xs[tok_idx])
                contrib = self.experts[e](sub)
            else:
                contrib = self.experts[e](x[tok_idx])
            out.index_add_(0, tok_idx, contrib * weights[tok_idx, k_idx, None])
        return out


class DecoderLayer(nn.Module):
    def __init__(self, cfg: ModelArchConfig, layer_idx: int):
        super().__init__()
        self.input_layernorm = nn.Parameter(torch.ones(cfg.hidden_size))
        self.post_attention_layernorm = nn.Parameter(torch.ones(cfg.hidden_size))
        self.self_attn = Attention(cfg, layer_idx)
        self.mlp = (
            MoEMLP(cfg) if cfg.num_local_experts > 0 else MLP(cfg, layer_idx)
        )
        self.eps = cfg.rms_norm_eps
        self.post_norms = cfg.post_norms
        self.res_mult = cfg.residual_multiplier or 1.0
        if cfg.post_norms:
            self.pre_feedforward_layernorm = nn.Parameter(
                torch.ones(cfg.hidden_size)
            )
            self.post_feedforward_layernorm = nn.Parameter(
                torch.ones(cfg.hidden_size)
            )

    def fp8_fused(self, fb, on_gpu: bool) -> bool:
        return (
            not self.post_norms
            and getattr(self, "_fp8_fused", False)
            and on_gpu
            and fb.lora_ids is None
        )

    def forward(self, x, residual, fb, kv_cache, cos_sin, normed=None):
        if self.post_norms:
            hidden = x if residual is None else x + residual
            a = self.self_attn(
                ops.rmsnorm(hidden, self.input_layernorm, self.eps),
                fb, kv_cache, cos_sin,
            )
            a = ops.rmsnorm(a, self.post_attention_layernorm, self.eps)
            h2 = hidden + a
            mm = self.mlp(
                ops.rmsnorm(h2, self.pre_feedforward_layernorm, self.eps), fb
            )
            mm = ops.rmsnorm(mm, self.post_feedforward_layernorm, self.eps)
            return mm, h2
        if self.fp8_fused(fb, x.is_cuda):
            if residual is None:
                residual = x
                if normed is not None:
                    xq, xs = normed
                else:
                    xq, xs = ops.rmsnorm_fp8(x, self.input_layernorm, self.eps)
            else:
                xq, xs = ops.fused_add_rmsnorm_fp8(
                    x, residual, self.input_layernorm, self.eps
                )
            x = self.self_attn((xq, xs), fb, kv_cache, cos_sin)
            if isinstance(self.mlp, MoEMLP):
                x, residual = ops.fused_add_rmsnorm(
                    x, residual, self.post_attention_layernorm, self.eps
                )
                x = self.mlp(x)
            else:
                xq, xs = ops.fused_add_rmsnorm_fp8(
                    x, residual, self.post_attention_layernorm, self.eps
                )
                x = self.mlp((xq, xs))
            return x, residual
        if residual is None:
            residual = x
            x = ops.rmsnorm(x, self.input_layernorm, self.eps)
        else:
            x, residual = ops.fused_add_rmsnorm(
                x, residual, self.input_layernorm, self.eps
            )
        x = self.self_attn(x, fb, kv_cache, cos_sin)
        if self.res_mult != 1.0:
            x = x * self.res_mult
        x, residual = ops.fused_add_rmsnorm(
            x, residual, self.post_attention_layernorm, self.eps
        )
        x = self.mlp(x, fb)
        if self.res_mult != 1.0:
            x = x * self.res_mult
        return x, residual


class LlamaForCausalLM(nn.Module):

    def __init__(self, cfg: ModelArchConfig, device=None, dtype=torch.bfloat16):
        super().__init__()
        self.cfg = cfg
        prev_dtype = torch.get_default_dtype()
        torch.set_default_dtype(dtype)
        try:
            with torch.device(device if device is not None else "cpu"):
                self.embed_tokens = nn.Embedding(cfg.vocab_size, cfg.hidden_size)
                self.layers = nn.ModuleList(
                    [DecoderLayer(cfg, i) for i in range(cfg.num_hidden_layers)]
                )
                self.norm = nn.Parameter(torch.ones(cfg.hidden_size))
                if cfg.tie_word_embeddings:
                    self.lm_head = None
                else:
                    self.lm_head = EngineLinear(
                        cfg.hidden_size, cfg.vocab_size, bias=False
                    )
        finally:
            torch.set_default_dtype(prev_dtype)
        from kubeai_amd.ops import ref as ops_ref

        self.register_buffer(
            "cos_sin",
            ops_ref.make_cos_sin_cache(
                cfg.head_dim, cfg.max_position_embeddings, cfg.rope_theta,
                rope_scaling=cfg.rope_scaling,
            ).to(device=device),
            persistent=False,
        )
        if cfg.rope_local_base_freq:
            self.register_buffer(
                "cos_sin_local",
                ops_ref.make_cos_sin_cache(
                    cfg.head_dim, cfg.max_position_embeddings,
                    cfg.rope_local_base_freq,
                ).to(device=device),
                persistent=False,
            )
        else:
            self.cos_sin_local = None

    def _decoder_stack(self, fb: ForwardBatch):
        cs = (
            (self.cos_sin, self.cos_sin_local)
            if self.cos_sin_local is not None
            else self.cos_sin
        )
        table = self.embed_tokens.weight
        l0 = self.layers[0]
        normed = None
        if (
            l0.fp8_fused(fb, table.is_cuda)
            and not self.cfg.scale_embeddings
            and not self.cfg.embedding_multiplier
            and fb.mm_embeds is None
        ):
            x, xq, xs = ops.embed_rmsnorm_fp8(
                fb.input_ids, table, l0.input_layernorm, l0.eps
            )
            normed = (xq, xs)
        else:
            x = self.embed_tokens(fb.input_ids.long())
            if self.cfg.scale_embeddings:
                x = x * torch.tensor(
                    self.cfg.hidden_size ** 0.5, dtype=x.dtype
                )
            elif self.cfg.embedding_multiplier:
                x = x * self.cfg.embedding_multiplier
            if fb.mm_embeds is not None:
                x = x.index_copy(0, fb.mm_idx, fb.mm_embeds.to(x.dtype))
        residual = None
        for i, layer in enumerate(self.layers):
            x, residual = layer(
                x, residual, fb, self.kv_caches[i], cs,
                normed=normed if i == 0 else None,
            )
        return x, residual

    @torch.inference_mode()
    def forward(self, fb: ForwardBatch) -> torch.Tensor:
        x, residual = self._decoder_stack(fb)
        x, _ = ops.fused_add_rmsnorm(x, residual, self.norm, self.cfg.rms_norm_eps)
        return x

    @torch.inference_mode()
    def forward_logits(self, fb: ForwardBatch, fp32: bool = True) -> torch.Tensor:
        from kubeai_amd.engine.quant import Fp8Linear

        x, residual = self._decoder_stack(fb)
        if isinstance(self.lm_head, Fp8Linear) and x.is_cuda:
            xq, xs = ops.fused_add_rmsnorm_fp8_div(
                x, residual, self.norm, self.cfg.rms_norm_eps
            )
            return self._finish_logits(
                self.lm_head.forward_quantized(xq, xs), fp32
            )
        x, _ = ops.fused_add_rmsnorm(x, residual, self.norm, self.cfg.rms_norm_eps)
        return self.compute_logits(x, fp32)

    @torch.inference_mode()
    def compute_logits(self, hidden: torch.Tensor, fp32: bool = True) -> torch.Tensor:
        if self.lm_head is None:
            logits = F.linear(hidden, self.embed_tokens.weight)
        else:
            logits = self.lm_head(hidden)
        return self._finish_logits(logits, fp32)

    def _finish_logits(self, logits: torch.Tensor, fp32: bool) -> torch.Tensor:
        if fp32 or self.cfg.logits_scaling or self.cfg.final_logit_softcap > 0:
            logits = logits.float()
        if self.cfg.logits_scaling:
            logits = logits / self.cfg.logits_scaling
        cap = self.cfg.final_logit_softcap
        if cap > 0:
            logits = cap * torch.tanh(logits / cap)
        return logits

    def bind_kv_caches(self, kv_caches: list[tuple[torch.Tensor, torch.Tensor]]):
        self.kv_caches = kv_caches
```

### kubeai_amd/ops/__init__.py

```python
from __future__ import annotations

import os
from typing import NamedTuple

import torch

from . import ref

_C = None
_C_IMPORT_ERROR: Exception | None = None
try:
    from kubeai_amd import _C
except Exception as e:
    _C_IMPORT_ERROR = e


def have_hip_ext() -> bool:
    return _C is not None


def _require_ext() -> None:
    if _C is None:
        raise RuntimeError(
            "kubeai_amd HIP extension (kubeai_amd._C) is not built but a GPU "
            "tensor reached the ops layer. Build it with "
            "`python setup.py build_ext --inplace` (PYTORCH_ROCM_ARCH=gfx950). "
            f"Original import error: {_C_IMPORT_ERROR!r}"
        )


def rmsnorm(x: torch.Tensor, weight: torch.Tensor, eps: float) -> torch.Tensor:
    if x.is_cuda:
        _require_ext()
        out = torch.empty_like(x)
        _C.rmsnorm(out, x, weight, eps)
        return out
    return ref.rmsnorm(x, weight, eps)


def fused_add_rmsnorm(x, residual, weight, eps: float):
    if x.is_cuda:
        _require_ext()
        _C.fused_add_rmsnorm(x, residual, weight, eps)
        return x, residual
    return ref.fused_add_rmsnorm(x, residual, weight, eps)


def rope(q, k, positions, cos_sin):
    if q.is_cuda:
        _require_ext()
        _C.rope(q, k, positions, cos_sin)
        return q, k
    return ref.rope(q, k, positions, cos_sin)


def reshape_and_cache(k, v, k_cache, v_cache, slot_mapping) -> None:
    if k.is_cuda:
        _require_ext()
        _C.reshape_and_cache(k, v, k_cache, v_cache, slot_mapping)
        return
    ref.reshape_and_cache(k, v, k_cache, v_cache, slot_mapping)


def rope_and_cache(q, k, v, positions, cos_sin, k_cache, v_cache, slot_mapping):
    if q.is_cuda:
        _require_ext()
        _C.rope_and_cache(
            q, k, v, positions, cos_sin, k_cache, v_cache, slot_mapping
        )
        return q, k
    q, k = ref.rope(q, k, positions, cos_sin)
    ref.reshape_and_cache(k, v, k_cache, v_cache, slot_mapping)
    return q, k


def paged_attention_decode(
    q, k_cache, v_cache, block_tables, seq_lens, scale: float, out=None,
    window: int = 0, softcap: float = 0.0, fp8_out: bool = False,
):
    if q.is_cuda:
        _require_ext()
        if out is None:
            out = torch.empty(q.shape, dtype=q.dtype, device=q.device)
        if fp8_out:
            B = q.shape[0]
            o8 = torch.empty(
                (B, q.shape[1] * q.shape[2]), dtype=torch.float8_e4m3fn,
                device=q.device,
            )
            oscale = torch.empty(B, dtype=torch.float32, device=q.device)
            _C.paged_attention_decode_fp8(
                out, o8, oscale, q, k_cache, v_cache, block_tables, seq_lens,
                scale, window, softcap
            )
            return out, o8, oscale
        _C.paged_attention_decode(
            out, q, k_cache, v_cache, block_tables, seq_lens, scale, window,
            softcap
        )
        return out
    res = ref.paged_attention_decode(
        q, k_cache, v_cache, block_tables, seq_lens, scale, window=window,
        softcap=softcap,
    )
    if out is not None:
        out.copy_(res)
        res = out
    if fp8_out:
        o8, oscale = ref.quant_fp8(res.reshape(res.shape[0], -1))
        return res, o8, oscale
    return res


def decode_rope_fused() -> bool:
    return os.environ.get("KUBEAI_DECODE_ROPE_FUSED", "1") != "0"


def rope_cache_attention_decode(
    q, k, v, positions, cos_sin, k_cache, v_cache, slot_mapping,
    block_tables, seq_lens, scale: float, out=None, window: int = 0,
    softcap: float = 0.0, fp8_out: bool = False,
):
    if q.is_cuda and decode_rope_fused():
        _require_ext()
        if out is None:
            out = torch.empty(q.shape, dtype=q.dtype, device=q.device)
        o8 = oscale = None
        if fp8_out:
            o8, oscale = _empty_fp8_rows(
                (q.shape[0], q.shape[1] * q.shape[2]), q.device
            )
        _C.rope_cache_attention_decode(
            out, o8, oscale, q, k, v, positions, cos_sin, k_cache, v_cache,
            slot_mapping, block_tables, seq_lens, scale, window, softcap
        )
        return (out, o8, oscale) if fp8_out else out
    if not q.is_cuda:
        res = ref.rope_cache_attention_decode(
            q, k, v, positions, cos_sin, k_cache, v_cache, slot_mapping,
            block_tables, seq_lens, scale, window=window, softcap=softcap,
        )
        if out is not None:
            out.copy_(res)
            res = out
        if fp8_out:
            o8, oscale = ref.quant_fp8(res.reshape(res.shape[0], -1))
            return res, o8, oscale
        return res
    qr, _ = rope_and_cache(
        q, k, v, positions, cos_sin, k_cache, v_cache, slot_mapping
    )
    return paged_attention_decode(
        qr, k_cache, v_cache, block_tables, seq_lens, scale, out=out,
        window=window, softcap=softcap, fp8_out=fp8_out,
    )


def paged_attention_prefill(
    q, k_cache, v_cache, block_tables, query_start_loc, seq_lens, scale: float,
    out=None, window: int = 0, softcap: float = 0.0,
):
    if q.is_cuda:
        _require_ext()
        if out is None:
            out = torch.empty(q.shape, dtype=q.dtype, device=q.device)
        _C.paged_attention_prefill(
            out, q, k_cache, v_cache, block_tables, query_start_loc, seq_lens,
            scale, window, softcap
        )
        return out
    res = ref.paged_attention_prefill(
        q, k_cache, v_cache, block_tables, query_start_loc, seq_lens, scale,
        window=window, softcap=softcap,
    )
    if out is not None:
        out.copy_(res)
        return out
    return res


def silu_and_mul(x):
    if x.is_cuda:
        _require_ext()
        T, two_i = x.shape
        out = torch.empty((T, two_i // 2), dtype=x.dtype, device=x.device)
        _C.silu_and_mul(out, x)
        return out
    return ref.silu_and_mul(x)


def gelu_and_mul(x):
    if x.is_cuda:
        _require_ext()
        T, two_i = x.shape
        out = torch.empty((T, two_i // 2), dtype=x.dtype, device=x.device)
        _C.gelu_and_mul(out, x)
        return out
    return ref.gelu_and_mul(x)


_USE_SKINNY = os.environ.get("KUBEAI_SKINNY_GEMM", "0") == "1"


def linear(x, weight):
    if (
        _USE_SKINNY
        and x.is_cuda
        and x.dtype == torch.bfloat16
        and x.dim() == 2
        and 1 <= x.shape[0] <= 64
        and weight.shape[1] % 64 == 0
        and weight.shape[0] % 64 == 0
        and x.is_contiguous()
        and weight.is_contiguous()
    ):
        _require_ext()
        y = torch.empty(
            (x.shape[0], weight.shape[0]), dtype=x.dtype, device=x.device
        )
        _C.skinny_gemm(y, x, weight)
        return y
    return torch.nn.functional.linear(x, weight)



INT4_M_FUSED = int(os.environ.get("KUBEAI_INT4_M_FUSED", "64"))

_INT4_WORKSPACE: dict = {}


def int4_reserve_workspace(device, numel: int) -> None:
    device = torch.device(device)
    ws = _INT4_WORKSPACE.get(device)
    if ws is None or ws.numel() < numel:
        _INT4_WORKSPACE[device] = torch.empty(
            numel, dtype=torch.bfloat16, device=device
        )


def int4_dequant(w, out=None):
    if not w.qp.is_cuda:
        res = w.dequant()
        if out is not None:
            out.copy_(res)
            return out
        return res
    _require_ext()
    if out is None:
        out = torch.empty((w.N, w.K), dtype=torch.bfloat16, device=w.qp.device)
    _C.int4_dequant(out, w.qp, w.sp, w.zp, w.N, w.K, w.group)
    return out


def int4_linear(x, w):
    if not x.is_cuda:
        return torch.nn.functional.linear(x, w.dequant())
    _require_ext()
    if x.dim() != 2:
        return int4_linear(x.reshape(-1, x.shape[-1]), w).view(*x.shape[:-1], w.N)
    M = x.shape[0]
    if 1 <= M <= min(INT4_M_FUSED, 64):
        if x.stride(1) != 1 or x.stride(0) % 8 or x.data_ptr() % 16:
            x = x.contiguous()
        y = torch.empty((M, w.N), dtype=torch.bfloat16, device=x.device)
        _C.int4_gemm(y, x, w.qp, w.sp, w.zp, w.N, w.K, w.group)
        return y
    ws = _INT4_WORKSPACE.get(x.device)
    if ws is None or ws.numel() < w.N * w.K:
        raise RuntimeError(
            "int4 workspace was not reserved for this weight "
            f"([{w.N}, {w.K}] on {x.device})"
        )
    dense = int4_dequant(w, out=ws[: w.N * w.K].view(w.N, w.K))
    return torch.nn.functional.linear(x, dense)



INT4_MOE_T = int(os.environ.get("KUBEAI_INT4_MOE_T", "64"))


def int4_moe_linear(x, selected, group, row_div: int, out=None):
    if not x.is_cuda:
        res = ref.moe_linear(
            x, selected, [w.dequant() for w in group.weights], row_div
        )
        if out is not None:
            out.copy_(res)
            return out
        return res
    _require_ext()
    if x.dim() == 2 and (x.stride(1) != 1 or x.stride(0) % 8 or x.data_ptr() % 16):
        x = x.contiguous()
    if out is None:
        out = torch.empty(
            (selected.numel(), group.N), dtype=torch.bfloat16, device=x.device
        )
    _C.int4_moe_gemm(
        out, x, selected, group.table_on(x.device), row_div, group.E, group.N,
        group.K, group.group,
    )
    return out


def moe_combine(y, selected, weights, n_experts: int | None = None):
    if not y.is_cuda:
        return ref.moe_combine(y, selected, weights, n_experts)
    _require_ext()
    out = torch.empty(
        (selected.shape[0], y.shape[1]), dtype=y.dtype, device=y.device
    )
    _C.moe_combine(out, y, selected, weights, n_experts or 0)
    return out


def int4_moe_mlp(x, selected, weights, gate_up_group, down_group):
    if not x.is_cuda:
        return ref.moe_mlp(
            x, selected, weights,
            [w.dequant() for w in gate_up_group.weights],
            [w.dequant() for w in down_group.weights],
        )
    h = int4_moe_linear(x, selected, gate_up_group, selected.shape[1])
    y = int4_moe_linear(silu_and_mul(h), selected, down_group, 1)
    return moe_combine(y, selected, weights, gate_up_group.E)


def _empty_fp8_rows(shape, device):
    out = torch.empty(shape, dtype=torch.float8_e4m3fn, device=device)
    scale = torch.empty(shape[0], dtype=torch.float32, device=device)
    return out, scale


def rmsnorm_fp8(x, weight, eps: float):
    _require_ext()
    out, scale = _empty_fp8_rows(x.shape, x.device)
    _C.rmsnorm_fp8(out, scale, x, weight, eps)
    return out, scale


def fused_add_rmsnorm_fp8(x, residual, weight, eps: float):
    _require_ext()
    out, scale = _empty_fp8_rows(x.shape, x.device)
    _C.fused_add_rmsnorm_fp8(out, scale, x, residual, weight, eps)
    return out, scale


def silu_and_mul_fp8(x):
    if not x.is_cuda:
        return ref.quant_fp8(ref.silu_and_mul(x))
    _require_ext()
    T, two_i = x.shape
    out, scale = _empty_fp8_rows((T, two_i // 2), x.device)
    _C.silu_and_mul_fp8(out, scale, x)
    return out, scale


def quant_fp8(x):
    if not x.is_cuda:
        return ref.quant_fp8(x)
    _require_ext()
    out, scale = _empty_fp8_rows(x.shape, x.device)
    _C.quant_fp8(out, scale, x)
    return out, scale


_QUANT_DIV_MAX_H = 32768


def quant_fp8_div(x):
    if (
        x.is_cuda
        and x.dtype == torch.bfloat16
        and x.dim() == 2
        and x.is_contiguous()
        and x.shape[1] % 8 == 0
        and 0 < x.shape[1] <= _QUANT_DIV_MAX_H
        and os.environ.get("KUBEAI_QUANT_DIV_KERNEL", "1") != "0"
    ):
        _require_ext()
        out, scale = _empty_fp8_rows(x.shape, x.device)
        _C.quant_fp8_div(out, scale, x)
        return out, scale.view(-1, 1)
    return ref.quant_fp8_div(x)


def _row_kernel_ok(x) -> bool:
    return (
        x.is_cuda
        and x.dtype == torch.bfloat16
        and x.dim() == 2
        and x.is_contiguous()
        and x.shape[1] % 8 == 0
        and 0 < x.shape[1] <= _QUANT_DIV_MAX_H
    )


def embed_rmsnorm_fp8(ids, table, weight, eps: float):
    if (
        _row_kernel_ok(table)
        and ids.is_cuda
        and ids.dtype == torch.int32
        and ids.dim() == 1
        and ids.is_contiguous()
        and weight.dtype == torch.bfloat16
    ):
        _require_ext()
        T, H = ids.shape[0], table.shape[1]
        x = torch.empty((T, H), dtype=table.dtype, device=table.device)
        out, scale = _empty_fp8_rows((T, H), table.device)
        _C.embed_rmsnorm_fp8(out, scale, x, ids, table, weight, eps)
        return x, out, scale
    x = torch.nn.functional.embedding(ids.long(), table)
    if x.is_cuda:
        return (x, *rmsnorm_fp8(x, weight, eps))
    return (x, *ref.quant_fp8(ref.rmsnorm(x, weight, eps)))


def fused_add_rmsnorm_fp8_div(x, residual, weight, eps: float,
                              write_rows: bool = False):
    if (
        _row_kernel_ok(x)
        and residual.is_contiguous()
        and residual.shape == x.shape
        and residual.dtype == x.dtype
        and weight.dtype == torch.bfloat16
    ):
        _require_ext()
        out, scale = _empty_fp8_rows(x.shape, x.device)
        _C.fused_add_rmsnorm_fp8_div(
            out, scale, x, residual, weight, eps, write_rows
        )
        return out, scale.view(-1, 1)
    y, _ = fused_add_rmsnorm(x, residual, weight, eps)
    return quant_fp8_div(y)


def greedy_sample(logits):
    if logits.is_cuda:
        _require_ext()
        out = torch.empty(logits.shape[0], dtype=torch.int64, device=logits.device)
        _C.greedy_sample(out, logits)
        return out
    return ref.greedy_sample(logits)


def gumbel_sample(logits, temperature, seeds, step: int):
    if logits.is_cuda:
        _require_ext()
        out = torch.empty(logits.shape[0], dtype=torch.int64, device=logits.device)
        _C.gumbel_sample(out, logits, temperature, seeds, step)
        return out
    return ref.gumbel_sample(logits, temperature, seeds, step)


class SampleResult(NamedTuple):

    tokens: torch.Tensor
    logprob: torch.Tensor
    lse: torch.Tensor
    packed: torch.Tensor | None = None


def _empty_sample_result(logits) -> SampleResult:
    B = logits.shape[0]
    packed = torch.empty(2 * B, dtype=torch.int64, device=logits.device)
    f = packed[B:].view(torch.float32)
    return SampleResult(packed[:B], f[:B], f[B:], packed)


def sample_to_host(res: SampleResult) -> tuple[list[int], list[float]]:
    if res.packed is None or not res.packed.is_cuda:
        return res.tokens.tolist(), res.logprob.tolist()
    B = res.tokens.shape[0]
    host = res.packed[: B + (B + 1) // 2].cpu()
    return host[:B].tolist(), host[B:].view(torch.float32)[:B].tolist()


def greedy_sample_logprob(logits) -> SampleResult:
    if logits.is_cuda:
        _require_ext()
        res = _empty_sample_result(logits)
        _C.greedy_sample_logprob(res.tokens, res.logprob, res.lse, logits)
        return res
    return SampleResult(*ref.greedy_sample_logprob(logits))


def gumbel_sample_logprob(logits, temperature, seeds, step: int) -> SampleResult:
    if logits.is_cuda:
        _require_ext()
        res = _empty_sample_result(logits)
        _C.gumbel_sample_logprob(
            res.tokens, res.logprob, res.lse, logits, temperature, seeds, step
        )
        return res
    return SampleResult(
        *ref.gumbel_sample_logprob(logits, temperature, seeds, step)
    )


def token_logprobs(logits, tokens):
    if logits.is_cuda:
        _require_ext()
        B = logits.shape[0]
        out = torch.empty((2, B), dtype=torch.float32, device=logits.device)
        _C.token_logprobs(out[0], out[1], logits, tokens)
        return out[0], out[1]
    return ref.token_logprobs(logits, tokens)


def nucleus_stats(logits, temps):
    if logits.is_cuda:
        _require_ext()
        S = logits.shape[0]
        m = torch.empty(S, dtype=torch.float32, device=logits.device)
        z = torch.empty_like(m)
        _C.nucleus_stats(m, z, logits, temps)
        return m, z
    t = temps.clamp_min(1e-6).unsqueeze(1)
    m = logits.max(dim=-1).values
    z = torch.exp((logits - m.unsqueeze(1)) / t).sum(-1)
    return m, z


def nucleus_accept(logits, cand, m, z, temps, top_ps, top_ks):
    if logits.is_cuda:
        _require_ext()
        ok = torch.empty(logits.shape[0], dtype=torch.uint8,
                         device=logits.device)
        _C.nucleus_accept(ok, logits, cand, m, z, temps, top_ps, top_ks)
        return ok
    t = temps.clamp_min(1e-6).unsqueeze(1)
    lt = logits.gather(1, cand.view(-1, 1))
    above = logits > lt
    mass = (torch.exp((logits - m.unsqueeze(1)) / t) * above).sum(-1) / z
    cnt = above.sum(-1)
    ok = (mass < top_ps) & ((top_ks <= 0) | (cnt < top_ks)) | (temps <= 0)
    return ok.to(torch.uint8)
```

Before: 7605 tok/s.

## Prefetch next fp8 weight into cache from extra blocks of preceding small kernels

```diff
diff --git a/kubeai_amd/csrc/attention_decode.hip b/kubeai_amd/csrc/attention_decode.hip
--- a/kubeai_amd/csrc/attention_decode.hip
+++ b/kubeai_amd/csrc/attention_decode.hip
@@ -6,6 +6,7 @@
 #include "attention_plan.h"
 #include "common.h"
 #include "dispatch.h"
+#include "prefetch_check.h"
 
 namespace {
 
@@ -482,7 +483,10 @@
     float* __restrict__ out_scale,
     const float* __restrict__ part_o,
     const float* __restrict__ part_ml,
-    const int n_q, const int n_splits) {
+    const int n_q, const int n_splits,
+    const void* __restrict__ pf_ptr, const int64_t pf_bytes,
+    const int pf_blocks) {
+  if (prefetch_block(pf_ptr, pf_bytes, pf_blocks)) return;
   __shared__ float red[16];
   const int b = blockIdx.x;
   const int row_len = n_q * HD;
@@ -530,7 +534,8 @@
 
 }
 
-void quant_fp8(torch::Tensor out, torch::Tensor out_scale, torch::Tensor x);
+void quant_fp8_with(torch::Tensor out, torch::Tensor out_scale, torch::Tensor x,
+                    const PrefetchArgs pf);
 
 namespace {
 
@@ -543,7 +548,7 @@
                  torch::Tensor k_cache, torch::Tensor v_cache,
                  torch::Tensor block_tables, torch::Tensor seq_lens,
                  double scale, int64_t window, double softcap,
-                 const RawQKV* raw = nullptr) {
+                 const RawQKV* raw = nullptr, const PrefetchArgs pf = {}) {
   const AttnShape s =
       check_paged_attention(out, q, k_cache, v_cache, block_tables, seq_lens);
   const int B = q.size(0), n_q = s.n_q, n_kv = s.n_kv, hd = s.hd;
@@ -634,7 +639,7 @@
   });
   HIP_CHECK_KERNEL();
   if (n_splits == 1) {
-    if (want_fp8) quant_fp8(*out_fp8, *out_scale, out.view({B, -1}));
+    if (want_fp8) quant_fp8_with(*out_fp8, *out_scale, out.view({B, -1}), pf);
     return;
   }
   static_assert(kMergeSplitCapHi == 16, "decode_n_splits caps splits at 16");
@@ -653,10 +658,10 @@
             (nvec + threads - 1) / threads, "merge pass count", [&](auto p) {
               hipLaunchKernelGGL(
                   (decode_merge_fp8_kernel<HD, decltype(p)::value, SCAP>),
-                  dim3(B), dim3(threads), 0, stream, (ushort*)out.data_ptr(),
-                  (unsigned char*)out_fp8->data_ptr(),
+                  dim3(B + pf.blocks), dim3(threads), 0, stream,
+                  (ushort*)out.data_ptr(), (unsigned char*)out_fp8->data_ptr(),
                   out_scale->data_ptr<float>(), part_o_ptr, part_ml_ptr, n_q,
-                  n_splits);
+                  n_splits, pf.ptr, pf.bytes, pf.blocks);
             });
       } else {
         const int64_t n_bh = (int64_t)B * n_q;
@@ -670,7 +675,8 @@
     });
   });
   HIP_CHECK_KERNEL();
-  if (want_fp8 && !fuse_fp8) quant_fp8(*out_fp8, *out_scale, out.view({B, -1}));
+  if (want_fp8 && !fuse_fp8)
+    quant_fp8_with(*out_fp8, *out_scale, out.view({B, -1}), pf);
 }
 
 }
@@ -688,9 +694,13 @@
                                 torch::Tensor k_cache, torch::Tensor v_cache,
                                 torch::Tensor block_tables,
                                 torch::Tensor seq_lens, double scale,
-                                int64_t window, double softcap) {
+                                int64_t window, double softcap,
+                                c10::optional<torch::Tensor> prefetch,
+                                int64_t prefetch_bytes,
+                                int64_t n_prefetch_blocks) {
   decode_impl(out, out_fp8, out_scale, q, k_cache, v_cache, block_tables,
-              seq_lens, scale, window, softcap);
+              seq_lens, scale, window, softcap, nullptr,
+              check_prefetch(prefetch, prefetch_bytes, n_prefetch_blocks, q));
 }
 
 void rope_cache_attention_decode(
@@ -699,8 +709,10 @@
     torch::Tensor v, torch::Tensor positions, torch::Tensor cos_sin,
     torch::Tensor k_cache, torch::Tensor v_cache, torch::Tensor slot_mapping,
     torch::Tensor block_tables, torch::Tensor seq_lens, double scale,
-    int64_t window, double softcap) {
+    int64_t window, double softcap, c10::optional<torch::Tensor> prefetch,
+    int64_t prefetch_bytes, int64_t n_prefetch_blocks) {
   const RawQKV raw{k, v, positions, cos_sin, slot_mapping};
   decode_impl(out, out_fp8, out_scale, q, k_cache, v_cache, block_tables,
-              seq_lens, scale, window, softcap, &raw);
-}
+              seq_lens, scale, window, softcap, &raw,
+              check_prefetch(prefetch, prefetch_bytes, n_prefetch_blocks, q));
+}
diff --git a/kubeai_amd/csrc/bindings.cpp b/kubeai_amd/csrc/bindings.cpp
--- a/kubeai_amd/csrc/bindings.cpp
+++ b/kubeai_amd/csrc/bindings.cpp
@@ -4,6 +4,7 @@
 #include <utility>
 
 #include "attention_plan.h"
+#include "prefetch_plan.h"
 
 void rmsnorm(torch::Tensor out, torch::Tensor x, torch::Tensor weight,
              double eps);
@@ -26,14 +27,18 @@
                                 torch::Tensor k_cache, torch::Tensor v_cache,
                                 torch::Tensor block_tables,
                                 torch::Tensor seq_lens, double scale,
-                                int64_t window, double softcap);
+                                int64_t window, double softcap,
+                                c10::optional<torch::Tensor> prefetch,
+                                int64_t prefetch_bytes,
+                                int64_t n_prefetch_blocks);
 void rope_cache_attention_decode(
     torch::Tensor out, c10::optional<torch::Tensor> out_fp8,
     c10::optional<torch::Tensor> out_scale, torch::Tensor q, torch::Tensor k,
     torch::Tensor v, torch::Tensor positions, torch::Tensor cos_sin,
     torch::Tensor k_cache, torch::Tensor v_cache, torch::Tensor slot_mapping,
     torch::Tensor block_tables, torch::Tensor seq_lens, double scale,
-    int64_t window, double softcap);
+    int64_t window, double softcap, c10::optional<torch::Tensor> prefetch,
+    int64_t prefetch_bytes, int64_t n_prefetch_blocks);
 void paged_attention_prefill(torch::Tensor out, torch::Tensor q,
                              torch::Tensor k_cache, torch::Tensor v_cache,
                              torch::Tensor block_tables,
@@ -80,20 +85,29 @@
 int64_t xgmi_max_elems();
 void xgmi_shutdown();
 void rmsnorm_fp8(torch::Tensor out, torch::Tensor out_scale, torch::Tensor x,
-                 torch::Tensor weight, double eps);
+                 torch::Tensor weight, double eps,
+                 c10::optional<torch::Tensor> prefetch, int64_t prefetch_bytes,
+                 int64_t n_prefetch_blocks);
 void fused_add_rmsnorm_fp8(torch::Tensor out, torch::Tensor out_scale,
                            torch::Tensor x, torch::Tensor residual,
-                           torch::Tensor weight, double eps);
+                           torch::Tensor weight, double eps,
+                           c10::optional<torch::Tensor> prefetch,
+                           int64_t prefetch_bytes, int64_t n_prefetch_blocks);
 void fused_add_rmsnorm_fp8_div(torch::Tensor out, torch::Tensor out_scale,
                                torch::Tensor x, torch::Tensor residual,
                                torch::Tensor weight, double eps,
                                bool write_rows);
 void embed_rmsnorm_fp8(torch::Tensor out, torch::Tensor out_scale,
                        torch::Tensor x_out, torch::Tensor ids,
-                       torch::Tensor table, torch::Tensor weight, double eps);
+                       torch::Tensor table, torch::Tensor weight, double eps,
+                       c10::optional<torch::Tensor> prefetch,
+                       int64_t prefetch_bytes, int64_t n_prefetch_blocks);
 void silu_and_mul_fp8(torch::Tensor out, torch::Tensor out_scale,
-                      torch::Tensor x);
-void quant_fp8(torch::Tensor out, torch::Tensor out_scale, torch::Tensor x);
+                      torch::Tensor x, c10::optional<torch::Tensor> prefetch,
+                      int64_t prefetch_bytes, int64_t n_prefetch_blocks);
+void quant_fp8(torch::Tensor out, torch::Tensor out_scale, torch::Tensor x,
+               c10::optional<torch::Tensor> prefetch, int64_t prefetch_bytes,
+               int64_t n_prefetch_blocks);
 void quant_fp8_div(torch::Tensor out, torch::Tensor out_scale,
                    torch::Tensor x);
 void nucleus_stats(torch::Tensor m, torch::Tensor z, torch::Tensor logits,
@@ -117,8 +131,28 @@
 static int64_t decode_plan(int64_t B, int64_t n_kv, int64_t max_blocks) {
   return attn_plan::decode_n_splits((int)B, (int)n_kv, (int)max_blocks);
 }
+static std::pair<int64_t, int64_t> prefetch_plan_slice(int64_t bytes,
+                                                       int64_t n_blocks,
+                                                       int64_t block,
+                                                       int64_t threads) {
+  TORCH_CHECK(bytes >= 0 && n_blocks >= 1 && block >= 0 && block < n_blocks &&
+              threads >= 1);
+  const prefetch_plan::Slice s = prefetch_plan::block_slice(
+      bytes, (int)n_blocks, (int)block, (int)threads);
+  return {s.begin, s.end};
+}
+
+#define PREFETCH_PYARGS                                  \
+  pybind11::arg("prefetch") = pybind11::none(),          \
+  pybind11::arg("prefetch_bytes") = 0, pybind11::arg("n_prefetch_blocks") = 0
 
 PYBIND11_MODULE(TORCH_EXTENSION_NAME, m) {
+  namespace py = pybind11;
+  m.def("prefetch_plan", &prefetch_plan_slice,
+        "(begin, end) bytes that extra block `block` of `n_blocks` streams "
+        "from a weight of `bytes` bytes in a `threads`-wide workgroup",
+        py::arg("bytes"), py::arg("n_blocks"), py::arg("block"),
+        py::arg("threads"));
   m.def("prefill_plan", &prefill_plan,
         "(version, waves per workgroup) paged_attention_prefill launches",
         pybind11::arg("Tq"), pybind11::arg("B"), pybind11::arg("n_q"),
@@ -140,10 +174,19 @@
   m.def("paged_attention_decode", &paged_attention_decode,
         "paged attention, one query token per seq");
   m.def("paged_attention_decode_fp8", &paged_attention_decode_fp8,
-        "paged decode attention that also emits the e4m3 row quant of out");
+        "paged decode attention that also emits the e4m3 row quant of out",
+        py::arg("out"), py::arg("out_fp8"), py::arg("out_scale"), py::arg("q"),
+        py::arg("k_cache"), py::arg("v_cache"), py::arg("block_tables"),
+        py::arg("seq_lens"), py::arg("scale"), py::arg("window"),
+        py::arg("softcap"), PREFETCH_PYARGS);
   m.def("rope_cache_attention_decode", &rope_cache_attention_decode,
         "pure-decode step: rotary embedding and KV cache write inside the "
-        "decode attention kernel (q, k, v are only read)");
+        "decode attention kernel (q, k, v are only read)",
+        py::arg("out"), py::arg("out_fp8"), py::arg("out_scale"), py::arg("q"),
+        py::arg("k"), py::arg("v"), py::arg("positions"), py::arg("cos_sin"),
+        py::arg("k_cache"), py::arg("v_cache"), py::arg("slot_mapping"),
+        py::arg("block_tables"), py::arg("seq_lens"), py::arg("scale"),
+        py::arg("window"), py::arg("softcap"), PREFETCH_PYARGS);
   m.def("paged_attention_prefill", &paged_attention_prefill,
         "paged causal flash attention over cached KV");
   m.def("gelu_and_mul", &gelu_and_mul, "GeGLU tanh-gelu(gate)*up");
@@ -180,16 +223,24 @@
         "temperature sampling + the token's logprob and the row logsumexp");
   m.def("token_logprobs", &token_logprobs,
         "logprob of given tokens and the row logsumexp, one launch");
-  m.def("rmsnorm_fp8", &rmsnorm_fp8, "rmsnorm with fused fp8 row quant");
+  m.def("rmsnorm_fp8", &rmsnorm_fp8, "rmsnorm with fused fp8 row quant",
+        py::arg("out"), py::arg("out_scale"), py::arg("x"), py::arg("weight"),
+        py::arg("eps"), PREFETCH_PYARGS);
   m.def("fused_add_rmsnorm_fp8", &fused_add_rmsnorm_fp8,
-        "residual add + rmsnorm with fused fp8 row quant");
+        "residual add + rmsnorm with fused fp8 row quant", py::arg("out"),
+        py::arg("out_scale"), py::arg("x"), py::arg("residual"),
+        py::arg("weight"), py::arg("eps"), PREFETCH_PYARGS);
   m.def("fused_add_rmsnorm_fp8_div", &fused_add_rmsnorm_fp8_div,
         "residual add + rmsnorm, then the division-form fp8 row quant of its "
         "bf16 row (lm_head's input)");
   m.def("embed_rmsnorm_fp8", &embed_rmsnorm_fp8,
-        "embedding gather + rmsnorm with fused fp8 row quant (layer 0)");
-  m.def("silu_and_mul_fp8", &silu_and_mul_fp8, "SwiGLU with fused fp8 quant");
-  m.def("quant_fp8", &quant_fp8, "bf16 -> fp8 row quant");
+        "embedding gather + rmsnorm with fused fp8 row quant (layer 0)",
+        py::arg("out"), py::arg("out_scale"), py::arg("x_out"), py::arg("ids"),
+        py::arg("table"), py::arg("weight"), py::arg("eps"), PREFETCH_PYARGS);
+  m.def("silu_and_mul_fp8", &silu_and_mul_fp8, "SwiGLU with fused fp8 quant",
+        py::arg("out"), py::arg("out_scale"), py::arg("x"), PREFETCH_PYARGS);
+  m.def("quant_fp8", &quant_fp8, "bf16 -> fp8 row quant", py::arg("out"),
+        py::arg("out_scale"), py::arg("x"), PREFETCH_PYARGS);
   m.def("quant_fp8_div", &quant_fp8_div,
         "bf16 -> fp8 row quant, division form (Fp8Linear.forward)");
   m.def("nucleus_stats", &nucleus_stats, "per-row softmax max + Z");
diff --git a/kubeai_amd/csrc/common.h b/kubeai_amd/csrc/common.h
--- a/kubeai_amd/csrc/common.h
+++ b/kubeai_amd/csrc/common.h
@@ -6,6 +6,8 @@
 #include <hip/hip_fp8.h>
 #include <stdint.h>
 #include <c10/hip/HIPStream.h>
+
+#include "prefetch_plan.h"
 
 #define WAVE_SIZE 64
 #define DEV_INLINE __device__ __forceinline__
@@ -184,6 +186,47 @@
   return *reinterpret_cast<uint2*>(packed);
 }
 
+DEV_INLINE void prefetch_slice(const void* __restrict__ p, const int64_t begin,
+                               const int64_t end) {
+  constexpr int kDepth = 8;
+  const int64_t total = end - begin;
+  if (total < prefetch_plan::kVecBytes) return;
+  const unsigned char* base = static_cast<const unsigned char*>(p) + begin;
+  const int64_t last = total - prefetch_plan::kVecBytes;
+  const uint32_t chunk = blockDim.x * (uint32_t)prefetch_plan::kVecBytes;
+  const uint32_t lane_off = threadIdx.x * (uint32_t)prefetch_plan::kVecBytes;
+  uint32_t acc = 0;
+#pragma unroll 1
+  for (int64_t done = 0; done < total; done += (int64_t)kDepth * chunk) {
+    const int64_t left = last - done;
+    const uint32_t lim = left < (int64_t)kDepth * chunk ? (uint32_t)left
+                                                        : kDepth * chunk;
+    const uint64_t pa = reinterpret_cast<uint64_t>(base + done);
+    const unsigned char* pass = reinterpret_cast<const unsigned char*>(
+        (uint64_t)__builtin_amdgcn_readfirstlane((uint32_t)(pa >> 32)) << 32 |
+        (uint32_t)__builtin_amdgcn_readfirstlane((uint32_t)pa));
+    uint4 r[kDepth];
+#pragma unroll
+    for (int k = 0; k < kDepth; ++k) {
+      const uint32_t off = k * chunk + lane_off;
+      r[k] = *reinterpret_cast<const uint4*>(pass + (off < lim ? off : lim));
+    }
+#pragma unroll
+    for (int k = 0; k < kDepth; ++k) acc |= r[k].x | r[k].y | r[k].z | r[k].w;
+    asm volatile("" ::"v"(acc));
+  }
+}
+
+DEV_INLINE bool prefetch_block(const void* __restrict__ p, const int64_t bytes,
+                               const int n_blocks) {
+  const int rows = (int)gridDim.x - n_blocks;
+  if ((int)blockIdx.x < rows) return false;
+  const prefetch_plan::Slice s = prefetch_plan::block_slice(
+      bytes, n_blocks, (int)blockIdx.x - rows, (int)blockDim.x);
+  prefetch_slice(p, s.begin, s.end);
+  return true;
+}
+
 DEV_INLINE float silu(const float x) { return x / (1.0f + __expf(-x)); }
 
 DEV_INLINE uint64_t splitmix64(uint64_t z) {
diff --git a/kubeai_amd/csrc/prefetch_check.h b/kubeai_amd/csrc/prefetch_check.h
--- /dev/null
+++ b/kubeai_amd/csrc/prefetch_check.h
@@ -0,0 +1,31 @@
+#pragma once
+
+#include <torch/extension.h>
+
+#include "prefetch_plan.h"
+
+struct PrefetchArgs {
+  const void* ptr = nullptr;
+  int64_t bytes = 0;
+  int blocks = 0;
+};
+
+constexpr int kPrefetchMaxBlocks = 1024;
+
+inline PrefetchArgs check_prefetch(const c10::optional<torch::Tensor>& t,
+                                   const int64_t nbytes, const int64_t n_blocks,
+                                   const torch::Tensor& like) {
+  if (!t.has_value()) return {};
+  TORCH_CHECK(t->is_contiguous(), "prefetch tensor is not contiguous");
+  TORCH_CHECK(t->device() == like.device(), "prefetch tensor is on ",
+              t->device(), ", the op runs on ", like.device());
+  TORCH_CHECK(nbytes >= 0 && nbytes <= (int64_t)t->nbytes(), "prefetch of ",
+              nbytes, " bytes from a tensor of ", t->nbytes());
+  TORCH_CHECK(n_blocks >= 0 && n_blocks <= kPrefetchMaxBlocks,
+              "prefetch block count ", n_blocks);
+  TORCH_CHECK(reinterpret_cast<uintptr_t>(t->data_ptr()) %
+                      prefetch_plan::kVecBytes == 0,
+              "prefetch tensor is not 16-byte aligned");
+  if (nbytes < prefetch_plan::kVecBytes || n_blocks == 0) return {};
+  return {t->data_ptr(), nbytes, (int)n_blocks};
+}
diff --git a/kubeai_amd/csrc/prefetch_plan.h b/kubeai_amd/csrc/prefetch_plan.h
--- /dev/null
+++ b/kubeai_amd/csrc/prefetch_plan.h
@@ -0,0 +1,31 @@
+#pragma once
+
+#include <cstdint>
+
+#ifdef __HIPCC__
+#define PREFETCH_PLAN_FN __host__ __device__ inline
+#else
+#define PREFETCH_PLAN_FN inline
+#endif
+
+namespace prefetch_plan {
+
+constexpr int64_t kVecBytes = 16;
+
+struct Slice {
+  int64_t begin, end;
+};
+
+PREFETCH_PLAN_FN Slice block_slice(const int64_t bytes, const int n_blocks,
+                                   const int block, const int threads) {
+  const int64_t total = bytes / kVecBytes * kVecBytes;
+  const int64_t chunk = (int64_t)threads * kVecBytes;
+  const int64_t n_chunks = (total + chunk - 1) / chunk;
+  int64_t begin = n_chunks * block / n_blocks * chunk;
+  int64_t end = n_chunks * (block + 1) / n_blocks * chunk;
+  if (begin > total) begin = total;
+  if (end > total) end = total;
+  return {begin, end};
+}
+
+}
diff --git a/kubeai_amd/csrc/row_kernels.hip b/kubeai_amd/csrc/row_kernels.hip
--- a/kubeai_amd/csrc/row_kernels.hip
+++ b/kubeai_amd/csrc/row_kernels.hip
@@ -4,6 +4,7 @@
 
 #include "common.h"
 #include "dispatch.h"
+#include "prefetch_check.h"
 
 namespace {
 
@@ -36,9 +37,13 @@
     const float eps, const int H,
     const int32_t* __restrict__ ids = nullptr,
     const int V = 0,
-    const bool write_rows = true) {
+    const bool write_rows = true,
+    const void* __restrict__ pf_ptr = nullptr, const int64_t pf_bytes = 0,
+    const int pf_blocks = 0) {
   static_assert(!kEmbed || (kFp8Out && !kFused && !kDiv));
   static_assert(!kDiv || (kFp8Out && kFused));
+  if constexpr (kFp8Out && !kDiv)
+    if (prefetch_block(pf_ptr, pf_bytes, pf_blocks)) return;
   const int row = blockIdx.x;
   int64_t src = row;
   if constexpr (kEmbed) src = min(max(ids[row], 0), V - 1);
@@ -166,7 +171,11 @@
     unsigned char* __restrict__ out,
     float* __restrict__ out_scale,
     const ushort* __restrict__ xin,
-    const int W) {
+    const int W,
+    const void* __restrict__ pf_ptr, const int64_t pf_bytes,
+    const int pf_blocks) {
+  if constexpr (!kDiv)
+    if (prefetch_block(pf_ptr, pf_bytes, pf_blocks)) return;
   const int row = blockIdx.x;
   const ushort* in = xin + (int64_t)row * Producer::kInWidth * W;
   const int nvec = W / 8;
@@ -218,7 +227,8 @@
 void launch_rmsnorm(void* out, float* out_scale, const torch::Tensor& x,
                     void* residual, const torch::Tensor& weight, double eps,
                     const torch::Tensor* ids = nullptr,
-                    const bool write_rows = true) {
+                    const bool write_rows = true,
+                    const PrefetchArgs pf = {}) {
   const int H = x.size(-1);
   check_row_op(x, H);
   const int T = kEmbed ? ids->numel() : x.numel() / H;
@@ -233,18 +243,19 @@
     constexpr int kIters = decltype(iters)::value;
     hipLaunchKernelGGL(
         (rmsnorm_kernel<kFused, kFp8Out, kThreads, kIters, kDiv, kEmbed>),
-        dim3(T), dim3(kThreads), 0, c10::hip::getCurrentHIPStream().stream(),
+        dim3(T + pf.blocks), dim3(kThreads), 0,
+        c10::hip::getCurrentHIPStream().stream(),
         (out_t*)out, out_scale, (ushort*)x.data_ptr(), (ushort*)residual,
         (const ushort*)weight.data_ptr(), (float)eps, H,
         kEmbed ? ids->data_ptr<int32_t>() : nullptr,
-        kEmbed ? (int)x.size(0) : 0, write_rows);
+        kEmbed ? (int)x.size(0) : 0, write_rows, pf.ptr, pf.bytes, pf.blocks);
   });
   HIP_CHECK_KERNEL();
 }
 
 template <typename Producer, bool kDiv = false>
 void launch_row_fp8(torch::Tensor& out, torch::Tensor& out_scale,
-                    const torch::Tensor& x) {
+                    const torch::Tensor& x, const PrefetchArgs pf = {}) {
   const int W = x.size(-1) / Producer::kInWidth;
   check_row_op(x, W);
   TORCH_CHECK(x.size(-1) == (int64_t)W * Producer::kInWidth);
@@ -253,12 +264,13 @@
   dispatch_row<RowPolicy::kMax>(W / 8, [&](auto threads, auto iters) {
     constexpr int kThreads = decltype(threads)::value;
     constexpr int kIters = decltype(iters)::value;
-    hipLaunchKernelGGL((row_fp8_kernel<Producer, kDiv, kThreads, kIters>), dim3(T),
-                       dim3(kThreads), 0,
+    hipLaunchKernelGGL((row_fp8_kernel<Producer, kDiv, kThreads, kIters>),
+                       dim3(T + pf.blocks), dim3(kThreads), 0,
                        c10::hip::getCurrentHIPStream().stream(),
                        (unsigned char*)out.data_ptr(),
                        out_scale.data_ptr<float>(),
-                       (const ushort*)x.data_ptr(), W);
+                       (const ushort*)x.data_ptr(), W, pf.ptr, pf.bytes,
+                       pf.blocks);
   });
   HIP_CHECK_KERNEL();
 }
@@ -279,17 +291,26 @@
 }
 
 void rmsnorm_fp8(torch::Tensor out, torch::Tensor out_scale, torch::Tensor x,
-                 torch::Tensor weight, double eps) {
+                 torch::Tensor weight, double eps,
+                 c10::optional<torch::Tensor> prefetch, int64_t prefetch_bytes,
+                 int64_t n_prefetch_blocks) {
+  const PrefetchArgs pf =
+      check_prefetch(prefetch, prefetch_bytes, n_prefetch_blocks, x);
   launch_rmsnorm<false, true>(out.data_ptr(), out_scale.data_ptr<float>(), x,
-                              nullptr, weight, eps);
+                              nullptr, weight, eps, nullptr, true, pf);
 }
 
 void fused_add_rmsnorm_fp8(torch::Tensor out, torch::Tensor out_scale,
                            torch::Tensor x, torch::Tensor residual,
-                           torch::Tensor weight, double eps) {
+                           torch::Tensor weight, double eps,
+                           c10::optional<torch::Tensor> prefetch,
+                           int64_t prefetch_bytes, int64_t n_prefetch_blocks) {
   TORCH_CHECK(residual.is_contiguous());
+  const PrefetchArgs pf =
+      check_prefetch(prefetch, prefetch_bytes, n_prefetch_blocks, x);
   launch_rmsnorm<true, true>(out.data_ptr(), out_scale.data_ptr<float>(), x,
-                             residual.data_ptr(), weight, eps);
+                             residual.data_ptr(), weight, eps, nullptr, true,
+                             pf);
 }
 
 void fused_add_rmsnorm_fp8_div(torch::Tensor out, torch::Tensor out_scale,
@@ -310,7 +331,9 @@
 
 void embed_rmsnorm_fp8(torch::Tensor out, torch::Tensor out_scale,
                        torch::Tensor x_out, torch::Tensor ids,
-                       torch::Tensor table, torch::Tensor weight, double eps) {
+                       torch::Tensor table, torch::Tensor weight, double eps,
+                       c10::optional<torch::Tensor> prefetch,
+                       int64_t prefetch_bytes, int64_t n_prefetch_blocks) {
   TORCH_CHECK(table.dim() == 2 && table.size(0) >= 1);
   TORCH_CHECK(ids.dim() == 1 && ids.is_contiguous() &&
               ids.scalar_type() == torch::kInt32);
@@ -322,18 +345,31 @@
   TORCH_CHECK(out_scale.is_contiguous() &&
               out_scale.scalar_type() == torch::kFloat32 &&
               out_scale.numel() == T);
+  const PrefetchArgs pf =
+      check_prefetch(prefetch, prefetch_bytes, n_prefetch_blocks, table);
   launch_rmsnorm<false, true, false, true>(
       out.data_ptr(), out_scale.data_ptr<float>(), table, x_out.data_ptr(),
-      weight, eps, &ids);
+      weight, eps, &ids, true, pf);
 }
 
 void silu_and_mul_fp8(torch::Tensor out, torch::Tensor out_scale,
-                      torch::Tensor x) {
-  launch_row_fp8<LoadSwiglu>(out, out_scale, x);
-}
-
-void quant_fp8(torch::Tensor out, torch::Tensor out_scale, torch::Tensor x) {
-  launch_row_fp8<LoadBf16>(out, out_scale, x);
+                      torch::Tensor x, c10::optional<torch::Tensor> prefetch,
+                      int64_t prefetch_bytes, int64_t n_prefetch_blocks) {
+  launch_row_fp8<LoadSwiglu>(
+      out, out_scale, x,
+      check_prefetch(prefetch, prefetch_bytes, n_prefetch_blocks, x));
+}
+
+void quant_fp8_with(torch::Tensor out, torch::Tensor out_scale, torch::Tensor x,
+                    const PrefetchArgs pf) {
+  launch_row_fp8<LoadBf16>(out, out_scale, x, pf);
+}
+
+void quant_fp8(torch::Tensor out, torch::Tensor out_scale, torch::Tensor x,
+               c10::optional<torch::Tensor> prefetch, int64_t prefetch_bytes,
+               int64_t n_prefetch_blocks) {
+  quant_fp8_with(out, out_scale, x,
+                 check_prefetch(prefetch, prefetch_bytes, n_prefetch_blocks, x));
 }
 
 void quant_fp8_div(torch::Tensor out, torch::Tensor out_scale,
diff --git a/kubeai_amd/models/llama.py b/kubeai_amd/models/llama.py
--- a/kubeai_amd/models/llama.py
+++ b/kubeai_amd/models/llama.py
@@ -9,6 +9,26 @@
 from kubeai_amd import ops
 from kubeai_amd.engine.batch import ForwardBatch
 from .config import ModelArchConfig
+
+
+PREFETCH_BLOCKS = 216
+PREFETCH_MAX_T = 64
+PREFETCH_BYTES = {"qkv": 0, "o": 16 << 20, "gate_up": 0, "down": 0}
+
+
+def weight_prefetch(site: str, proj, fb: ForwardBatch, T: int):
+    budget = PREFETCH_BYTES[site]
+    if (
+        budget <= 0
+        or not 0 < T <= PREFETCH_MAX_T
+        or fb.n_prefill != 0
+        or fb.n_decode != T
+    ):
+        return None
+    w = getattr(proj, "weight_fp8", None)
+    if w is None or not w.is_cuda:
+        return None
+    return w, min(budget, w.numel() * w.element_size()), PREFETCH_BLOCKS
 
 
 class EngineLinear(nn.Linear):
@@ -41,6 +61,7 @@
     window: int,
     softcap: float,
     fp8_out: bool,
+    o_proj=None,
 ):
     k_cache, v_cache = kv_cache
     T = q.shape[0]
@@ -63,6 +84,7 @@
             window=window,
             softcap=softcap,
             fp8_out=fp8_out,
+            prefetch=weight_prefetch("o", o_proj, fb, T) if fp8_out else None,
         )
         return res[1:] if fp8_out else out.view(T, -1)
     q, k = ops.rope_and_cache(
@@ -161,6 +183,7 @@
         attn = paged_attention_step(
             q, k, v, fb, kv_cache, cos_sin, scale=self.scale,
             window=self.window, softcap=self.softcap, fp8_out=fp8_in,
+            o_proj=self.o_proj,
         )
         if fp8_in:
             return self.o_proj.forward_quantized(*attn)
@@ -186,7 +209,10 @@
     def forward(self, x, fb: ForwardBatch | None = None) -> torch.Tensor:
         if isinstance(x, tuple):
             h = self.gate_up_proj.forward_quantized(*x)
-            a8, ascale = ops.silu_and_mul_fp8(h)
+            pf = None
+            if fb is not None:
+                pf = weight_prefetch("down", self.down_proj, fb, h.shape[0])
+            a8, ascale = ops.silu_and_mul_fp8(h, prefetch=pf)
             return self.down_proj.forward_quantized(a8, ascale)
         h = self.gate_up_proj(x)
         lm = getattr(self, "_lora_manager", None)
@@ -321,15 +347,19 @@
             mm = ops.rmsnorm(mm, self.post_feedforward_layernorm, self.eps)
             return mm, h2
         if self.fp8_fused(fb, x.is_cuda):
+            T = x.shape[0]
+            pf = weight_prefetch("qkv", self.self_attn.qkv_proj, fb, T)
             if residual is None:
                 residual = x
                 if normed is not None:
                     xq, xs = normed
                 else:
-                    xq, xs = ops.rmsnorm_fp8(x, self.input_layernorm, self.eps)
+                    xq, xs = ops.rmsnorm_fp8(
+                        x, self.input_layernorm, self.eps, prefetch=pf
+                    )
             else:
                 xq, xs = ops.fused_add_rmsnorm_fp8(
-                    x, residual, self.input_layernorm, self.eps
+                    x, residual, self.input_layernorm, self.eps, prefetch=pf
                 )
             x = self.self_attn((xq, xs), fb, kv_cache, cos_sin)
             if isinstance(self.mlp, MoEMLP):
@@ -339,9 +369,12 @@
                 x = self.mlp(x)
             else:
                 xq, xs = ops.fused_add_rmsnorm_fp8(
-                    x, residual, self.post_attention_layernorm, self.eps
+                    x, residual, self.post_attention_layernorm, self.eps,
+                    prefetch=weight_prefetch(
+                        "gate_up", self.mlp.gate_up_proj, fb, T
+                    ),
                 )
-                x = self.mlp((xq, xs))
+                x = self.mlp((xq, xs), fb)
             return x, residual
         if residual is None:
             residual = x
@@ -422,7 +455,10 @@
             and fb.mm_embeds is None
         ):
             x, xq, xs = ops.embed_rmsnorm_fp8(
-                fb.input_ids, table, l0.input_layernorm, l0.eps
+                fb.input_ids, table, l0.input_layernorm, l0.eps,
+                prefetch=weight_prefetch(
+                    "qkv", l0.self_attn.qkv_proj, fb, fb.input_ids.shape[0]
+                ),
             )
             normed = (xq, xs)
         else:
diff --git a/kubeai_amd/ops/__init__.py b/kubeai_amd/ops/__init__.py
--- a/kubeai_amd/ops/__init__.py
+++ b/kubeai_amd/ops/__init__.py
@@ -29,6 +29,17 @@
         )
 
 
+
+PREFETCH_BLOCKS = 216
+
+
+def _prefetch_args(prefetch) -> tuple:
+    if prefetch is None:
+        return None, 0, 0
+    tensor, nbytes, *rest = prefetch
+    return tensor, int(nbytes), int(rest[0]) if rest else PREFETCH_BLOCKS
+
+
 def rmsnorm(x: torch.Tensor, weight: torch.Tensor, eps: float) -> torch.Tensor:
     if x.is_cuda:
         _require_ext()
@@ -77,6 +88,7 @@
 def paged_attention_decode(
     q, k_cache, v_cache, block_tables, seq_lens, scale: float, out=None,
     window: int = 0, softcap: float = 0.0, fp8_out: bool = False,
+    prefetch=None,
 ):
     if q.is_cuda:
         _require_ext()
@@ -91,7 +103,7 @@
             oscale = torch.empty(B, dtype=torch.float32, device=q.device)
             _C.paged_attention_decode_fp8(
                 out, o8, oscale, q, k_cache, v_cache, block_tables, seq_lens,
-                scale, window, softcap
+                scale, window, softcap, *_prefetch_args(prefetch)
             )
             return out, o8, oscale
         _C.paged_attention_decode(
@@ -119,7 +131,7 @@
 def rope_cache_attention_decode(
     q, k, v, positions, cos_sin, k_cache, v_cache, slot_mapping,
     block_tables, seq_lens, scale: float, out=None, window: int = 0,
-    softcap: float = 0.0, fp8_out: bool = False,
+    softcap: float = 0.0, fp8_out: bool = False, prefetch=None,
 ):
     if q.is_cuda and decode_rope_fused():
         _require_ext()
@@ -132,7 +144,8 @@
             )
         _C.rope_cache_attention_decode(
             out, o8, oscale, q, k, v, positions, cos_sin, k_cache, v_cache,
-            slot_mapping, block_tables, seq_lens, scale, window, softcap
+            slot_mapping, block_tables, seq_lens, scale, window, softcap,
+            *_prefetch_args(prefetch if fp8_out else None)
         )
         return (out, o8, oscale) if fp8_out else out
     if not q.is_cuda:
@@ -152,7 +165,7 @@
     )
     return paged_attention_decode(
         qr, k_cache, v_cache, block_tables, seq_lens, scale, out=out,
-        window=window, softcap=softcap, fp8_out=fp8_out,
+        window=window, softcap=softcap, fp8_out=fp8_out, prefetch=prefetch,
     )
 
 
@@ -331,36 +344,38 @@
     return out, scale
 
 
-def rmsnorm_fp8(x, weight, eps: float):
+def rmsnorm_fp8(x, weight, eps: float, prefetch=None):
     _require_ext()
     out, scale = _empty_fp8_rows(x.shape, x.device)
-    _C.rmsnorm_fp8(out, scale, x, weight, eps)
+    _C.rmsnorm_fp8(out, scale, x, weight, eps, *_prefetch_args(prefetch))
     return out, scale
 
 
-def fused_add_rmsnorm_fp8(x, residual, weight, eps: float):
+def fused_add_rmsnorm_fp8(x, residual, weight, eps: float, prefetch=None):
     _require_ext()
     out, scale = _empty_fp8_rows(x.shape, x.device)
-    _C.fused_add_rmsnorm_fp8(out, scale, x, residual, weight, eps)
+    _C.fused_add_rmsnorm_fp8(
+        out, scale, x, residual, weight, eps, *_prefetch_args(prefetch)
+    )
     return out, scale
 
 
-def silu_and_mul_fp8(x):
+def silu_and_mul_fp8(x, prefetch=None):
     if not x.is_cuda:
         return ref.quant_fp8(ref.silu_and_mul(x))
     _require_ext()
     T, two_i = x.shape
     out, scale = _empty_fp8_rows((T, two_i // 2), x.device)
-    _C.silu_and_mul_fp8(out, scale, x)
+    _C.silu_and_mul_fp8(out, scale, x, *_prefetch_args(prefetch))
     return out, scale
 
 
-def quant_fp8(x):
+def quant_fp8(x, prefetch=None):
     if not x.is_cuda:
         return ref.quant_fp8(x)
     _require_ext()
     out, scale = _empty_fp8_rows(x.shape, x.device)
-    _C.quant_fp8(out, scale, x)
+    _C.quant_fp8(out, scale, x, *_prefetch_args(prefetch))
     return out, scale
 
 
@@ -395,7 +410,7 @@
     )
 
 
-def embed_rmsnorm_fp8(ids, table, weight, eps: float):
+def embed_rmsnorm_fp8(ids, table, weight, eps: float, prefetch=None):
     if (
         _row_kernel_ok(table)
         and ids.is_cuda
@@ -408,11 +423,13 @@
         T, H = ids.shape[0], table.shape[1]
         x = torch.empty((T, H), dtype=table.dtype, device=table.device)
         out, scale = _empty_fp8_rows((T, H), table.device)
-        _C.embed_rmsnorm_fp8(out, scale, x, ids, table, weight, eps)
+        _C.embed_rmsnorm_fp8(
+            out, scale, x, ids, table, weight, eps, *_prefetch_args(prefetch)
+        )
         return x, out, scale
     x = torch.nn.functional.embedding(ids.long(), table)
     if x.is_cuda:
-        return (x, *rmsnorm_fp8(x, weight, eps))
+        return (x, *rmsnorm_fp8(x, weight, eps, prefetch=prefetch))
     return (x, *ref.quant_fp8(ref.rmsnorm(x, weight, eps)))
 
 
```

After: 7473 tok/s. -1.7%, worse.
